# underactuated/HSLabs

Measured on AMD Instinct MI355X. Metric: batched control-loop steps/sec (hexapod.xml, 18-DoF) at 1/2/4/8 MI355X, higher is better.
Workload: dtype f64

## Files before the change

hslabs_amd/api.py:

```python
from __future__ import annotations

import ctypes
from dataclasses import dataclass, field

import numpy as np

from . import capi

GAIT_DTYPE = np.dtype([
    ("torso_pos", "<f8", (3,)), ("torso_angles", "<f8", (3,)), ("step_duration", "<f8"),
    ("period", "<f8"), ("step_length", "<f8"), ("step_height", "<f8"), ("curvature", "<f8"),
    ("foot_shift", "<f8"), ("foot_shift_type", "<i4"), ("rec_transform_flag", "<i4"),
    ("rec_transl", "<f8", (3,)), ("rec_eas", "<f8", (3,)), ("reserved", "<f8", (5,)),
])
assert GAIT_DTYPE.itemsize == 192


def _require(ok: bool, msg: str) -> None:
    if not ok:
        raise ValueError(msg)


def _torch_stream(device, stream):
    import torch
# ... 51 lines not shown
        r["step_length"] = self.step_length
        r["step_height"] = self.step_height
        r["curvature"] = self.curvature
        r["foot_shift_type"] = self.foot_shift[0]
        r["foot_shift"] = self.foot_shift[1]
        if self.rec_transform is not None:
            r["rec_transform_flag"] = 1
            r["rec_transl"] = self.rec_transform[0]
            r["rec_eas"] = self.rec_transform[1]
        return r

    @staticmethod
    def from_record(r) -> "PgsConfigParams":
        return PgsConfigParams(
            torso_pos=tuple(float(v) for v in r["torso_pos"]),
            torso_angles=tuple(float(v) for v in r["torso_angles"]),
            step_duration=float(r["step_duration"]), period=float(r["period"]),
            step_length=float(r["step_length"]), step_height=float(r["step_height"]),
            curvature=float(r["curvature"]), foot_shift=(int(r["foot_shift_type"]), float(r["foot_shift"])),
            rec_transform=((tuple(float(v) for v in r["rec_transl"]), tuple(float(v) for v in r["rec_eas"]))
                           if int(r["rec_transform_flag"]) else None))


def read_pgs_config(path: str, setup_id: int) -> PgsConfigParams:
    L = capi.load()
    c = capi.GaitParamsC()
    buf = ctypes.create_string_buffer(256)
    capi.check(L.hs_pgs_config_read(path.encode(), setup_id, ctypes.byref(c), buf, 256), "hs_pgs_config_read")
    rec = np.frombuffer(bytes(c), dtype=GAIT_DTYPE)[0]
    p = PgsConfigParams.from_record(rec)
    p.fname = buf.value.decode()
    return p


@dataclass
class KinematicModel:

    xml_path: str
    lik_variant: int = -1
    handle: ctypes.c_void_p = field(default=None, repr=False)

    def __post_init__(self):
        L = capi.load()
        h = ctypes.c_void_p()
        capi.check(L.hs_model_load_ex(self.xml_path.encode(), self.lik_variant, ctypes.byref(h)),
                   f"hs_model_load({self.xml_path})")
        self.handle = h
        d = capi.ModelDimsC()
        capi.check(L.hs_model_get_dims(h, ctypes.byref(d)), "hs_model_get_dims")
        self.n_parts, self.nmj, self.nfeet = d.n_parts, d.nmj, d.nfeet
        self.config_dim, self.n_limbs, self.lik_kind = d.config_dim, d.n_limbs, d.lik_kind
        self.total_mass, self.rcap = d.total_mass, d.rcap
        ok = ctypes.c_int32()
        capi.check(L.hs_model_limb_lane(h, ctypes.byref(ok)), "hs_model_limb_lane")
        self.limb_lane_ok = bool(ok.value)

    def get_config_dim(self) -> int:
        return self.config_dim

    def switch_torso_penalty(self, force: bool, torque: bool):
        capi.check(capi.load().hs_model_set_torso_penalty(self.handle, int(bool(force)), int(bool(torque))),
                   "hs_model_set_torso_penalty")

    def torso_penalty(self) -> tuple:
        f, t = ctypes.c_int32(), ctypes.c_int32()
        capi.check(capi.load().hs_model_get_torso_penalty(self.handle, ctypes.byref(f), ctypes.byref(t)),
                   "hs_model_get_torso_penalty")
        return bool(f.value), bool(t.value)

    def number_of_motor_joints(self) -> int:
        return self.nmj

    def get_mnode(self, i: int) -> dict:
        c = capi.NodeInfoC()
        capi.check(capi.load().hs_model_get_node(self.handle, i, ctypes.byref(c)), "hs_model_get_node")
        return {"parent": c.parent, "jtype": c.jtype, "hinge": c.hinge, "foot": c.foot, "limb": c.limb,
                "kids": list(c.kids[:c.n_kids]), "com": np.array(c.com), "foot_pos": np.array(c.foot_pos),
                "mass": c.mass}

    def pergen_rec(self, params, times) -> np.ndarray:
        arr = params_array(params)
        t = np.ascontiguousarray(times, dtype=np.float64).reshape(-1)
        rec = np.zeros((len(arr), len(t), 6 + 3 * self.n_limbs))
        dp = ctypes.POINTER(ctypes.c_double)
        capi.check(capi.load().hs_pergen_rec_host(self.handle, arr.ctypes.data_as(ctypes.POINTER(capi.GaitParamsC)),
                                                  len(arr), t.ctypes.data_as(dp), len(t), rec.ctypes.data_as(dp)),
                   "hs_pergen_rec_host")
        return rec

    def set_jvalues_with_lik(self, rec, ignore_reach: bool = False, config=None):
        r = np.ascontiguousarray(rec, dtype=np.float64).reshape(-1, 6 + 3 * self.n_limbs)
        n = len(r)
        q = np.zeros((n, self.config_dim)) if config is None else np.array(config, np.float64).reshape(n, -1)
        st = np.zeros(n, np.uint32)
        dp = ctypes.POINTER(ctypes.c_double)
        capi.check(capi.load().hs_model_lik_host(self.handle, n, r.ctypes.data_as(dp), int(ignore_reach),
                                                 q.ctypes.data_as(dp), st.ctypes.data_as(ctypes.POINTER(ctypes.c_uint32))),
                   "hs_model_lik_host")
        return q, st

    def recompute_modelnodes(self, config, joints: bool = False):
        q = np.ascontiguousarray(config, dtype=np.float64).reshape(-1, self.config_dim)
        n = len(q)
        ag = np.zeros((n, self.n_parts, 12))
        aj = np.zeros((n, self.n_parts, 12)) if joints else None
        dp = ctypes.POINTER(ctypes.c_double)
        capi.check(capi.load().hs_model_fk_host(self.handle, n, q.ctypes.data_as(dp), self.config_dim,
                                                ag.ctypes.data_as(dp), None if aj is None else aj.ctypes.data_as(dp)),
                   "hs_model_fk_host")

        def rows(a):
            return a.reshape(n, self.n_parts, 4, 3).transpose(0, 1, 3, 2).copy()
        return (rows(ag), rows(aj)) if joints else rows(ag)

    def __del__(self):
        try:
            if self.handle:
                capi.load().hs_model_free(self.handle)
                self.handle = None
        except Exception:
            pass


def limb_tile_launches() -> int:
    return int(capi.load().hs_limb_tile_launches())


def limb_tile_plan_launches() -> int:
    return int(capi.load().hs_limb_tile_plan_launches())


def limb_tile_loop_launches() -> int:
    return int(capi.load().hs_limb_tile_loop_launches())


def limb_launches() -> int:
    return int(capi.load().hs_limb_launches())


def limb_deferred() -> int:
    d = ctypes.c_int64()
    capi.check(capi.load().hs_limb_stats(None, ctypes.byref(d)), "hs_limb_stats")
    return int(d.value)


def limb_tables(model, rollout: int, n_rows: int, device=None, stream=None) -> dict:
    out = dict(ktab=np.zeros((n_rows, 6, 3)), kvel=np.zeros((n_rows, 6, 3)), kbig=np.zeros((n_rows, 6), np.uint8),
               kbad=np.zeros((n_rows, 6), np.uint8))
    dt = ctypes.c_double()
    capi.check(capi.load().hs_debug_limb_tables(model.handle, _cuda_stream(device, stream), rollout, n_rows,
                                                *(out[k].ctypes.data for k in ("ktab", "kvel", "kbig", "kbad")),
                                                ctypes.addressof(dt)), "hs_debug_limb_tables")
    out["dt"] = float(dt.value)
    return out


def params_array(params) -> np.ndarray:
    if isinstance(params, np.ndarray) and params.dtype == GAIT_DTYPE:
        return np.ascontiguousarray(params)
    arr = np.zeros(len(params), GAIT_DTYPE)
    for i, p in enumerate(params):
        arr[i] = p.to_record()
    return arr


def run_host(model: KinematicModel, params, n_t: int = 20, k0: int = 0, horizon: int | None = None,
             ignore_reach: bool = True, want=("q", "tau", "cf", "x", "flags", "work_cot")) -> dict:
    arr = params_array(params)
    B = len(arr)
    H = n_t if horizon is None else horizon
    shapes = _out_shapes(model, B, H)
    out = {k: np.zeros(shapes[k], np.uint32 if k == "flags" else np.float64) if k in want else None
           for k in ("q", "tau", "cf", "x", "flags", "work_cot")}
    dp = ctypes.POINTER(ctypes.c_double)

    def P(a, t=dp):
        return None if a is None else a.ctypes.data_as(t)

    L = capi.load()
    rc = L.hs_run_host(model.handle, arr.ctypes.data_as(ctypes.POINTER(capi.GaitParamsC)), B, n_t, k0, H,
                       int(ignore_reach), P(out["q"]), P(out["tau"]), P(out["cf"]), P(out["x"]),
                       P(out["flags"], ctypes.POINTER(ctypes.c_uint32)), P(out["work_cot"]))
    capi.check(rc, "hs_run_host")
    return out


class ShardedBatch:

    def __init__(self, model: KinematicModel, params, horizon: int = 1, n_t: int = 20, fp32: bool = False,
                 device_mask: int = 1):
        self.model = model
        self.params = params_array(params)
        self.B, self.H, self.n_t = len(self.params), horizon, n_t
        self.dtype = np.float32 if fp32 else np.float64
        L = capi.load()
        h = ctypes.c_void_p()
        capi.check(L.hs_batch_create(model.handle, self.B, horizon, n_t, capi.HS_PREC_F32 if fp32 else capi.HS_PREC_F64,
                                     device_mask, ctypes.byref(h)), "hs_batch_create")
        self.handle = h
        capi.check(L.hs_batch_set_params(h, self.params.ctypes.data_as(ctypes.POINTER(capi.GaitParamsC))),
                   "hs_batch_set_params")

    def _shapes(self) -> dict:
        shapes = _out_shapes(self.model, self.B, self.H)
        return {k: shapes[k] for k, _ in capi.BatchOutputsC._fields_}

    def run(self, k0: int = 0, ignore_reach: bool = True, want=("tau", "cf", "flags", "work", "cot")) -> dict:
        shapes = self._shapes()
        out = {k: np.zeros(shapes[k], np.uint32 if k == "flags" else self.dtype) for k in want}
        o = capi.BatchOutputsC(**{k: v.ctypes.data for k, v in out.items()})
        capi.check(capi.load().hs_batch_run(self.handle, k0, int(ignore_reach), ctypes.byref(o)), "hs_batch_run")
        return out

    def run_device(self, out: dict, k0: int = 0, ignore_reach: bool = True) -> None:
        import torch

        shapes = self._shapes()
        fdt = torch.float32 if self.dtype == np.float32 else torch.float64
        for k, v in out.items():
            if k not in shapes:
                raise ValueError(f"run_device: unknown output {k!r} (expected one of {sorted(shapes)})")
            if not isinstance(v, torch.Tensor) or not v.is_cuda:
                raise ValueError(f"run_device: {k} must be a GPU tensor")
            want = (torch.int32, torch.uint32) if k == "flags" else (fdt,)
            if v.dtype not in want:
                raise ValueError(f"run_device: {k} has dtype {v.dtype}, expected {' or '.join(map(str, want))}")
            if tuple(v.shape) != shapes[k]:
                raise ValueError(f"run_device: {k} has shape {tuple(v.shape)}, expected {shapes[k]}")
            if not v.is_contiguous():
                raise ValueError(f"run_device: {k} must be contiguous")
        o = capi.BatchOutputsC(**{k: v.data_ptr() for k, v in out.items()})
        capi.check(capi.load().hs_batch_run_device(self.handle, k0, int(ignore_reach), ctypes.byref(o)),
                   "hs_batch_run_device")

    def select_best(self, comm: "Comm | None" = None):
        c, i = ctypes.c_float(), ctypes.c_int64()
        L = capi.load()
        if comm is None:
            capi.check(L.hs_select_best(self.handle, ctypes.byref(c), ctypes.byref(i)), "hs_select_best")
        else:
            capi.check(L.hs_select_best_comm(self.handle, comm.handle, ctypes.byref(c), ctypes.byref(i)),
                       "hs_select_best_comm")
        return c.value, i.value

    def __del__(self):
        h = getattr(self, "handle", None)
        if h and capi._lib is not None:
            capi._lib.hs_batch_free(h)
            self.handle = None


class Comm:

    def __init__(self, n_ranks: int, rank: int, uid: bytes):
        _require(len(uid) == capi.COMM_ID_BYTES, f"a comm id is {capi.COMM_ID_BYTES} bytes")
        h = ctypes.c_void_p()
        capi.check(capi.load().hs_comm_init(n_ranks, rank, uid, ctypes.byref(h)), "hs_comm_init")
        self.handle, self.n_ranks, self.rank = h, n_ranks, rank

    @staticmethod
    def unique_id() -> bytes:
        buf = ctypes.create_string_buffer(capi.COMM_ID_BYTES)
        capi.check(capi.load().hs_comm_unique_id(buf), "hs_comm_unique_id")
        return buf.raw

    def reduce_best(self, key, stream=None) -> None:
        capi.check(capi.load().hs_comm_reduce_best(self.handle, key.data_ptr(), _cuda_stream(key.device, stream)),
                   "hs_comm_reduce_best")

    def free(self) -> None:
        if self.handle:
            capi.load().hs_comm_free(self.handle)
            self.handle = None

    def __del__(self):
        try:
            self.free()
        except Exception:
            pass


class DeviceBatch:

    def __init__(self, model: KinematicModel, params, n_t: int = 20, k0: int = 0, horizon: int = 1,
                 ignore_reach: bool = True, outputs=("tau", "cf", "work_cot", "flags"), device=None,
                 rollout_id_base: int = 0, dtype=None):
        import torch

        self.torch = torch
        self.model = model
        self._alloc(model, params, n_t, k0, horizon, ignore_reach, outputs, device, rollout_id_base, dtype)

    def _alloc(self, dims, params, n_t, k0, horizon, ignore_reach, outputs, device, rollout_id_base, dtype=None):
        torch = self.torch
        arr = params_array(params)
        self.B, self.H, self.n_t, self.k0 = len(arr), horizon, n_t, k0
        self.ignore_reach = ignore_reach
        self.rollout_id_base = rollout_id_base
        dev = device or torch.device("cuda", torch.cuda.current_device())
        self.device = dev
        self.dtype = dtype or torch.float64
        self.precision = _precision(self.dtype)
        self.params = torch.from_numpy(arr.view(np.uint8).copy()).to(dev)
        shapes = _out_shapes(dims, self.B, self.H)
        for k in ("q", "dq", "tau", "cf", "x", "flags", "work_cot"):
            setattr(self, k, torch.empty(shapes[k], dtype=torch.int32 if k == "flags" else self.dtype, device=dev)
# ... 663 lines not shown
```

hslabs_amd/capi.py:

```python
from __future__ import annotations

import ctypes
import hashlib
import os

from . import build as _build

ABI_VERSION = 16

HS_OK = 0
HS_FLAG_RANK_RETRY = 1
HS_FLAG_FULL_RANK = 2
HS_FLAG_LOOP_EXHAUST = 4
HS_FLAG_NAN = 8
HS_FLAG_UNREACH = 16
HS_FLAG_NO_CONTACT = 32
HS_FLAG_GENERAL = 64
HS_FLAG_NEAR_RANK = 256
HS_FLAG_DEPENDENT = 512
HS_PREC_F64 = 0
HS_PREC_F32 = 1
HS_SOLVE_AUTO = 0
HS_SOLVE_REFERENCE = 1
KEY_MIN_STEP_LENGTH = 1e-3
COMM_ID_BYTES = 128

EXPORTS = [
    "hs_model_load", "hs_model_load_ex", "hs_model_free", "hs_model_get_dims", "hs_pgs_config_read",
    "hs_run", "hs_run_steps", "hs_run_calls", "hs_run_pd", "hs_run_forces", "hs_run_forces_calls", "hs_mixed_create", "hs_mixed_free",
    "hs_mixed_get_dims", "hs_complete_traj", "hs_traj_save", "hs_run_forces_host",
    "hs_run_mixed", "hs_run_mixed_steps", "hs_run_mixed_calls", "hs_run_host", "hs_best_key_cot", "hs_best_key_encode",
    "hs_best_key_decode", "hs_last_error", "hs_abi_version",
    "hs_sim_default_params", "hs_sim_reset", "hs_sim_step", "hs_sim_create", "hs_sim_advance", "hs_sim_get_state",
    "hs_sim_free", "hs_sim_trial", "hs_sim_trial_summary", "hs_sim_set_trial", "hs_sim_get_trial_state",
    "hs_sim_config", "hs_sim_track_push", "hs_sim_probe", "hs_sim_estimate_workspace",
    "hs_cpc_default_params", "hs_cpc_torques", "hs_cpc_target_points", "hs_sim_cpc_workspace", "hs_sim_cpc_step",
    "hs_batch_create", "hs_batch_set_params", "hs_batch_run", "hs_batch_run_device", "hs_select_best",
    "hs_batch_best_key_device", "hs_batch_free", "hs_comm_unique_id", "hs_comm_init", "hs_comm_free", "hs_comm_size",
    "hs_comm_reduce_best", "hs_select_best_comm", "hs_pergen_rec", "hs_pergen_rec_host", "hs_model_lik",
    "hs_model_lik_host", "hs_model_fk", "hs_model_fk_host", "hs_model_get_node", "hs_model_set_torso_penalty",
    "hs_model_get_torso_penalty", "hs_model_limb_lane", "hs_limb_launches", "hs_limb_tile_launches", "hs_limb_stats",
    "hs_limb_tile_plan_launches", "hs_limb_tile_loop_launches", "hs_debug_limb_tables",
]
EXPORTS_B = ["hs_sim_regress_B", "hs_sim_estimate_B"]
HS_FLAG_LIK_FAILED = 128
SIM_BODY_STRIDE = 13
HS_TRIAL_RUNNING = -1
HS_TRIAL_SURVIVED = -2
HS_CPC_FLAG_NONFINITE = 1
HS_CPC_FLAG_NOSCORE = 2
HS_CPC_FLAG_RANK = 4


class GaitParamsC(ctypes.Structure):

    _fields_ = [
        ("torso_pos", ctypes.c_double * 3),
        ("torso_angles", ctypes.c_double * 3),
        ("step_duration", ctypes.c_double),
        ("period", ctypes.c_double),
        ("step_length", ctypes.c_double),
        ("step_height", ctypes.c_double),
        ("curvature", ctypes.c_double),
        ("foot_shift", ctypes.c_double),
        ("foot_shift_type", ctypes.c_int32),
        ("rec_transform_flag", ctypes.c_int32),
        ("rec_transl", ctypes.c_double * 3),
        ("rec_eas", ctypes.c_double * 3),
        ("reserved", ctypes.c_double * 5),
    ]


assert ctypes.sizeof(GaitParamsC) == 192


class BatchOutputsC(ctypes.Structure):

    _fields_ = [(f, ctypes.c_void_p) for f in ("q", "tau", "cf", "x", "flags", "work", "cot")]


class ModelDimsC(ctypes.Structure):
    _fields_ = [
        ("n_parts", ctypes.c_int32), ("nmj", ctypes.c_int32), ("nfeet", ctypes.c_int32),
        ("config_dim", ctypes.c_int32), ("n_limbs", ctypes.c_int32), ("lik_kind", ctypes.c_int32),
        ("total_mass", ctypes.c_double), ("rcap", ctypes.c_double),
    ]


class NodeInfoC(ctypes.Structure):
    _fields_ = [(f, ctypes.c_int32) for f in ("parent", "jtype", "hinge", "foot", "limb", "n_kids")] + \
               [("kids", ctypes.c_int32 * 6), ("com", ctypes.c_double * 3), ("foot_pos", ctypes.c_double * 3),
                ("mass", ctypes.c_double)]


class PdArgsC(ctypes.Structure):
    _fields_ = [("q_meas", ctypes.c_void_p), ("dq_meas", ctypes.c_void_p), ("k", ctypes.c_double),
                ("tau_cmd", ctypes.c_void_p), ("q_target", ctypes.c_void_p), ("dq_target", ctypes.c_void_p)]


class RunArgsC(ctypes.Structure):
    _fields_ = [
        ("n_rollouts", ctypes.c_int32), ("horizon", ctypes.c_int32), ("k0", ctypes.c_int32),
        ("n_t", ctypes.c_int32), ("ignore_reach", ctypes.c_int32), ("accumulate", ctypes.c_int32),
        ("params", ctypes.c_void_p), ("q", ctypes.c_void_p), ("tau", ctypes.c_void_p),
        ("cf", ctypes.c_void_p), ("x", ctypes.c_void_p), ("flags", ctypes.c_void_p),
        ("work_cot", ctypes.c_void_p), ("best_key", ctypes.c_void_p),
        ("rollout_id_base", ctypes.c_int64), ("stream", ctypes.c_void_p), ("dq", ctypes.c_void_p),
        ("precision", ctypes.c_int32), ("solve_mode", ctypes.c_int32), ("key_steps", ctypes.c_int32),
    ]


class SimParamsC(ctypes.Structure):
    _fields_ = [(f, ctypes.c_double) for f in ("dt", "k", "sor_w", "erp", "cfm", "gravity", "bounce", "bounce_vel",
                                               "soft_cfm", "mu")] + [("iterations", ctypes.c_int32),
                                                                     ("reserved", ctypes.c_int32)]


class SimArgsC(ctypes.Structure):
    _fields_ = [("n_rollouts", ctypes.c_int32), ("n_steps", ctypes.c_int32), ("n_t", ctypes.c_int32),
                ("precision", ctypes.c_int32), ("params", SimParamsC)] + \
               [(f, ctypes.c_void_p) for f in ("body", "seed", "tsi", "q_tab", "dq_tab", "tau_tab", "tau_cmd", "q_meas",
                                               "torso", "n_contacts", "normal_force", "stream")]


class SimTrialArgsC(ctypes.Structure):
    _fields_ = [("sim", SimArgsC)] + \
               [(f, ctypes.c_int32) for f in ("open_loop", "kick_every", "kick_phase", "check_from", "check_until",
                                              "reserved")] + \
               [("torque_limit", ctypes.c_double), ("hc", ctypes.c_double), ("kick_dv", ctypes.c_void_p),
                ("state", ctypes.c_void_p), ("fall_z", ctypes.c_void_p)]


class SimProbeArgsC(ctypes.Structure):
    _fields_ = [("n_rollouts", ctypes.c_int32), ("m", ctypes.c_int32), ("precision", ctypes.c_int32),
                ("reserved", ctypes.c_int32), ("params", SimParamsC)] + \
               [(f, ctypes.c_void_p) for f in ("body", "seed", "tau0", "dtau", "config_out", "tau_out", "body_out",
                                               "n_contacts", "stream")]


class SimEstimateArgsC(ctypes.Structure):
    _fields_ = [("probe", SimProbeArgsC)] + \
               [(f, ctypes.c_void_p) for f in ("ders", "U", "Bt", "rank", "workspace")] + \
               [("workspace_bytes", ctypes.c_size_t)]


class CpcParamsC(ctypes.Structure):
    _fields_ = [(f, ctypes.c_double) for f in ("w", "sg", "k0", "kc", "tauc", "loss_cc", "tp_dist")] + \
               [("n_cand", ctypes.c_int32), ("goal_t0s", ctypes.c_int32), ("tpdist_switch", ctypes.c_int32),
                ("mask", ctypes.c_uint32)]


class CpcArgsC(ctypes.Structure):
    _fields_ = [("n_rollouts", ctypes.c_int32), ("n_tp", ctypes.c_int32), ("precision", ctypes.c_int32),
                ("reserved", ctypes.c_int32), ("params", CpcParamsC), ("Bt", ctypes.c_void_p),
                ("state", ctypes.c_void_p), ("state_stride", ctypes.c_int64), ("tp", ctypes.c_void_p),
                ("tp_stride", ctypes.c_int64)] + \
               [(f, ctypes.c_void_p) for f in ("low_tpdist", "tau", "last_tpi", "flags", "loss", "cand_tpi", "cand_t0s",
                                               "passes", "i_best", "stream")]


class SimCpcArgsC(ctypes.Structure):
    _fields_ = [("trial", SimTrialArgsC), ("cpc", CpcParamsC), ("m", ctypes.c_int32), ("n_tp", ctypes.c_int32),
                ("dtau", ctypes.c_void_p), ("dtau_step_stride", ctypes.c_int64), ("tp", ctypes.c_void_p),
                ("tp_stride", ctypes.c_int64)] + \
               [(f, ctypes.c_void_p) for f in ("ders", "tau0", "low_tpdist", "last_tpi", "flags", "rank", "workspace")] + \
               [("workspace_bytes", ctypes.c_size_t)]


class TrialSummaryC(ctypes.Structure):
    _fields_ = [("running", ctypes.c_int32), ("survived", ctypes.c_int32), ("fallen", ctypes.c_int32),
                ("min_fall_tsi", ctypes.c_int32), ("sum_fall_tsi", ctypes.c_int64)]


C_STRUCTS = {
    "hs_gait_params": GaitParamsC, "hs_model_dims": ModelDimsC, "hs_node_info": NodeInfoC, "hs_run_args": RunArgsC,
    "hs_pd_args": PdArgsC, "hs_batch_outputs": BatchOutputsC, "hs_sim_params": SimParamsC, "hs_sim_args": SimArgsC,
    "hs_sim_trial_args": SimTrialArgsC, "hs_trial_summary": TrialSummaryC, "hs_sim_probe_args": SimProbeArgsC,
    "hs_sim_estimate_args": SimEstimateArgsC, "hs_cpc_params": CpcParamsC, "hs_cpc_args": CpcArgsC,
    "hs_sim_cpc_args": SimCpcArgsC,
}


class HSError(RuntimeError):
    pass


_lib = None
LOADED = None


def lib_path() -> str:
    return _build.LIB


def load(build_if_missing: bool = True) -> ctypes.CDLL:
    global _lib
    if _lib is not None:
        return _lib
    try:
        import torch
    except ImportError:
        pass
    path = _build.LIB
    variant = os.environ.get("HSLABS_VARIANT")
    if variant:
        if not variant.replace("_", "").isalnum():
            raise HSError(f"bad HSLABS_VARIANT {variant!r}")
        path = os.path.join(_build.VARIANT_DIR, f"libhslabs_{variant}.so")
        if not os.path.exists(path):
            raise HSError(f"HSLABS_VARIANT={variant}: {path} not built")
    if not os.path.exists(path):
        if not build_if_missing:
            raise HSError(f"libhslabs.so not built ({path}); run `python -m hslabs_amd.build`")
        _build.build()
    L = ctypes.CDLL(path)
    global LOADED
    with open(path, "rb") as f:
        LOADED = {"path": os.path.relpath(path, os.path.dirname(_build.HERE)),
                  "sha256": hashlib.sha256(f.read()).hexdigest()[:16]}
    dp = ctypes.POINTER(ctypes.c_double)
    vp = ctypes.c_void_p
    L.hs_model_load.argtypes = [ctypes.c_char_p, ctypes.POINTER(vp)]
    L.hs_model_load_ex.argtypes = [ctypes.c_char_p, ctypes.c_int, ctypes.POINTER(vp)]
    L.hs_model_free.argtypes = [vp]
    L.hs_model_free.restype = None
    L.hs_model_get_dims.argtypes = [vp, ctypes.POINTER(ModelDimsC)]
    L.hs_model_set_torso_penalty.argtypes = [vp, ctypes.c_int32, ctypes.c_int32]
    L.hs_model_get_torso_penalty.argtypes = [vp, ctypes.POINTER(ctypes.c_int32), ctypes.POINTER(ctypes.c_int32)]
    L.hs_pgs_config_read.argtypes = [ctypes.c_char_p, ctypes.c_int, ctypes.POINTER(GaitParamsC),
                                     ctypes.c_char_p, ctypes.c_int32]
    L.hs_run.argtypes = [vp, ctypes.POINTER(RunArgsC)]
    L.hs_run_steps.argtypes = [vp, ctypes.POINTER(RunArgsC), ctypes.c_int32, ctypes.POINTER(vp)]
    L.hs_run_calls.argtypes = [vp, ctypes.POINTER(RunArgsC), ctypes.c_int32]
    L.hs_run_mixed_calls.argtypes = [vp, ctypes.POINTER(RunArgsC), ctypes.c_int32]
    L.hs_run_forces.argtypes = [vp, ctypes.POINTER(RunArgsC), vp]
    L.hs_run_forces_calls.argtypes = [vp, ctypes.POINTER(RunArgsC), ctypes.c_int32, vp]
    L.hs_run_forces_host.argtypes = [vp, ctypes.POINTER(GaitParamsC), ctypes.c_int32, ctypes.c_int32, ctypes.c_int32,
                                     ctypes.c_int32, ctypes.c_int32, ctypes.POINTER(ctypes.c_double),
                                     ctypes.POINTER(ctypes.c_double), ctypes.POINTER(ctypes.c_uint32)]
    L.hs_run_pd.argtypes = [vp, ctypes.POINTER(RunArgsC), ctypes.POINTER(PdArgsC)]
    L.hs_complete_traj.argtypes = [vp, ctypes.POINTER(GaitParamsC), ctypes.c_int32, ctypes.c_int32, ctypes.c_int32,
                                   ctypes.POINTER(ctypes.c_double)]
    L.hs_traj_save.argtypes = [ctypes.c_char_p, ctypes.POINTER(ctypes.c_double), ctypes.c_int32, ctypes.c_int32,
                               ctypes.c_int32]
    L.hs_mixed_create.argtypes = [ctypes.POINTER(vp), ctypes.c_int32, ctypes.POINTER(ctypes.c_int32), ctypes.c_int32,
                                  ctypes.POINTER(vp)]
    L.hs_mixed_free.argtypes = [vp]
    L.hs_mixed_free.restype = None
    L.hs_mixed_get_dims.argtypes = [vp, ctypes.POINTER(ModelDimsC)]
    L.hs_run_mixed.argtypes = [vp, ctypes.POINTER(RunArgsC)]
    L.hs_run_mixed_steps.argtypes = [vp, ctypes.POINTER(RunArgsC), ctypes.c_int32, ctypes.POINTER(vp)]
    L.hs_run_host.argtypes = [vp, ctypes.POINTER(GaitParamsC), ctypes.c_int32, ctypes.c_int32, ctypes.c_int32,
                              ctypes.c_int32, ctypes.c_int32, dp, dp, dp, dp, ctypes.POINTER(ctypes.c_uint32), dp]
    L.hs_best_key_cot.argtypes = [ctypes.c_double, ctypes.c_double, ctypes.c_double, ctypes.c_int32, ctypes.c_int32]
    L.hs_best_key_cot.restype = ctypes.c_double
    L.hs_best_key_encode.argtypes = [ctypes.c_double, ctypes.c_int64]
    L.hs_best_key_encode.restype = ctypes.c_uint64
    L.hs_best_key_decode.argtypes = [ctypes.c_uint64, ctypes.POINTER(ctypes.c_float), ctypes.POINTER(ctypes.c_int64)]
    L.hs_best_key_decode.restype = None
    L.hs_sim_default_params.argtypes = [ctypes.POINTER(SimParamsC)]
    L.hs_sim_default_params.restype = None
    L.hs_sim_reset.argtypes = [vp, ctypes.c_int32, vp, ctypes.c_int32, vp, ctypes.c_int32, vp]
    L.hs_sim_step.argtypes = [vp, ctypes.POINTER(SimArgsC)]
    L.hs_sim_create.argtypes = [vp, ctypes.POINTER(GaitParamsC), ctypes.c_int32, ctypes.POINTER(SimParamsC),
                                ctypes.c_double, ctypes.POINTER(vp)]
    L.hs_sim_advance.argtypes = [vp, ctypes.c_int32, dp, dp, dp, ctypes.POINTER(ctypes.c_int32), dp]
    L.hs_sim_get_state.argtypes = [vp, dp, ctypes.POINTER(ctypes.c_int32)]
    L.hs_sim_free.argtypes = [vp]
    L.hs_sim_trial.argtypes = [vp, ctypes.POINTER(SimTrialArgsC)]
    L.hs_sim_trial_summary.argtypes = [vp, ctypes.c_int32, ctypes.POINTER(TrialSummaryC), vp]
    L.hs_sim_set_trial.argtypes = [vp, ctypes.c_int32, ctypes.c_double, ctypes.c_int32, ctypes.c_int32, dp,
                                   ctypes.c_double, ctypes.c_int32, ctypes.c_int32]
    L.hs_sim_get_trial_state.argtypes = [vp, ctypes.POINTER(ctypes.c_int32)]
    L.hs_sim_free.restype = None
    L.hs_sim_config.argtypes = [vp, ctypes.c_int32, vp, vp, ctypes.c_int32, ctypes.c_int32, vp]
    L.hs_sim_track_push.argtypes = [vp, ctypes.c_int32, vp, ctypes.c_int32, ctypes.c_double, vp, ctypes.c_int32, vp]
    L.hs_sim_probe.argtypes = [vp, ctypes.POINTER(SimProbeArgsC)]
    L.hs_sim_regress_B.argtypes = [vp, ctypes.c_int32, ctypes.c_int32, vp, vp, vp, vp, ctypes.c_int32, vp]
    L.hs_sim_estimate_workspace.argtypes = [vp, ctypes.c_int32, ctypes.c_int32]
    L.hs_sim_estimate_workspace.restype = ctypes.c_size_t
    L.hs_sim_estimate_B.argtypes = [vp, ctypes.POINTER(SimEstimateArgsC)]
    L.hs_cpc_default_params.argtypes = [ctypes.POINTER(CpcParamsC)]
    L.hs_cpc_default_params.restype = None
    L.hs_cpc_torques.argtypes = [vp, ctypes.POINTER(CpcArgsC)]
    L.hs_cpc_target_points.argtypes = [vp, ctypes.c_int32, ctypes.c_int32, vp, vp, vp, ctypes.c_uint32, vp, vp]
    L.hs_sim_cpc_workspace.argtypes = [vp, ctypes.c_int32, ctypes.c_int32]
    L.hs_sim_cpc_workspace.restype = ctypes.c_size_t
    L.hs_sim_cpc_step.argtypes = [vp, ctypes.POINTER(SimCpcArgsC)]
    L.hs_batch_create.argtypes = [vp, ctypes.c_int32, ctypes.c_int32, ctypes.c_int32, ctypes.c_int32, ctypes.c_uint32,
                                  ctypes.POINTER(vp)]
    L.hs_batch_set_params.argtypes = [vp, ctypes.POINTER(GaitParamsC)]
    L.hs_batch_run.argtypes = [vp, ctypes.c_int32, ctypes.c_int32, ctypes.POINTER(BatchOutputsC)]
    L.hs_batch_run_device.argtypes = [vp, ctypes.c_int32, ctypes.c_int32, ctypes.POINTER(BatchOutputsC)]
    L.hs_select_best.argtypes = [vp, ctypes.POINTER(ctypes.c_float), ctypes.POINTER(ctypes.c_int64)]
    L.hs_select_best_comm.argtypes = [vp, vp, ctypes.POINTER(ctypes.c_float), ctypes.POINTER(ctypes.c_int64)]
    L.hs_comm_unique_id.argtypes = [ctypes.c_char_p]
    L.hs_comm_init.argtypes = [ctypes.c_int32, ctypes.c_int32, ctypes.c_char_p, ctypes.POINTER(vp)]
    L.hs_comm_free.argtypes = [vp]
    L.hs_comm_free.restype = None
    L.hs_comm_size.argtypes = [vp, ctypes.POINTER(ctypes.c_int32), ctypes.POINTER(ctypes.c_int32)]
    L.hs_comm_reduce_best.argtypes = [vp, vp, vp]
    L.hs_batch_best_key_device.argtypes = [vp, ctypes.c_int32]
    L.hs_batch_best_key_device.restype = vp
    L.hs_batch_free.argtypes = [vp]
    L.hs_batch_free.restype = None
    u32p = ctypes.POINTER(ctypes.c_uint32)
    L.hs_pergen_rec.argtypes = [vp, vp, ctypes.c_int32, vp, ctypes.c_int32, vp, vp]
    L.hs_pergen_rec_host.argtypes = [vp, ctypes.POINTER(GaitParamsC), ctypes.c_int32, dp, ctypes.c_int32, dp]
    L.hs_model_lik.argtypes = [vp, ctypes.c_int32, vp, ctypes.c_int32, vp, vp, vp]
    L.hs_model_lik_host.argtypes = [vp, ctypes.c_int32, dp, ctypes.c_int32, dp, u32p]
    L.hs_model_fk.argtypes = [vp, ctypes.c_int32, vp, ctypes.c_int32, vp, vp, vp]
    L.hs_model_fk_host.argtypes = [vp, ctypes.c_int32, dp, ctypes.c_int32, dp, dp]
    L.hs_model_get_node.argtypes = [vp, ctypes.c_int32, ctypes.POINTER(NodeInfoC)]
    L.hs_last_error.argtypes = []
    L.hs_last_error.restype = ctypes.c_char_p
    L.hs_model_limb_lane.argtypes = [vp, ctypes.POINTER(ctypes.c_int32)]
    L.hs_limb_launches.argtypes = []
    L.hs_limb_launches.restype = ctypes.c_int64
    L.hs_limb_tile_launches.argtypes = []
    L.hs_limb_tile_launches.restype = ctypes.c_int64
    L.hs_limb_tile_plan_launches.argtypes = []
    L.hs_limb_tile_plan_launches.restype = ctypes.c_int64
    L.hs_limb_tile_loop_launches.argtypes = []
    L.hs_limb_tile_loop_launches.restype = ctypes.c_int64
    L.hs_debug_limb_tables.argtypes = [vp, vp, ctypes.c_int32, ctypes.c_int32, vp, vp, vp, vp, vp]
    L.hs_debug_limb_tables.restype = ctypes.c_int
    L.hs_limb_stats.argtypes = [ctypes.POINTER(ctypes.c_int64), ctypes.POINTER(ctypes.c_int64)]
    L.hs_abi_version.argtypes = []
    L.hs_abi_version.restype = ctypes.c_int
    if L.hs_abi_version() != ABI_VERSION:
        raise HSError("libhslabs ABI version mismatch")
    _lib = L
    return L


def check(rc: int, what: str = "") -> None:
    if rc != HS_OK:
        msg = load().hs_last_error().decode(errors="replace")
        raise HSError(f"{what}: {msg} (rc={rc})")
```

hslabs_amd/csrc/hs_capi.cpp:

```cpp
#include <hip/hip_runtime.h>

#include <algorithm>
#include <atomic>
#include <cmath>
#include <cstdio>
#include <cstdlib>
#include <cfloat>
#include <cstring>
#include <fstream>
#include <mutex>
#include <string>
#include <vector>

#include "hs_internal.h"

namespace {

thread_local std::string g_err;

int fail(int code, const std::string& msg) {
  g_err = msg;
  return code;
}

// ... 114 lines not shown
    hs_simtopo_t<float> h;
    hs_simtopo_round(h, m->sim);
    hs_simtopo_t<float>* d = nullptr;
    e = hipMalloc(&d, sizeof(h));
    if (e != hipSuccess) return failed(e, "hipMalloc(simtopo f32)");
    e = hipMemcpy(d, &h, sizeof(h), hipMemcpyHostToDevice);
    if (e != hipSuccess) { (void)hipFree(d); return failed(e, "hipMemcpy(simtopo f32)"); }
    m->sim_dev_f32[dev] = d;
  }
  dv.sim = m->sim_dev[dev];
  if (precision == HS_PREC_F32) dv.sim_f32 = m->sim_dev_f32[dev];
  return dv;
}

hs_run_args routed(const hs_run_args& a, int32_t torso_mask) {
  hs_run_args c = a;
  if (torso_mask != 3) c.solve_mode = HS_SOLVE_REFERENCE;
  return c;
}

int check_args(const hs_model_s* m, const hs_run_args* a) {
  if (!m || !a) return fail(HS_E_ARG, "null model or args");
  if (a->n_rollouts < 0) return fail(HS_E_ARG, "n_rollouts < 0");
  if (a->horizon < 1) return fail(HS_E_ARG, "horizon must be >= 1");
  if (a->k0 < 0) return fail(HS_E_ARG, "k0 must be >= 0");
  if (a->precision != HS_PREC_F64 && a->precision != HS_PREC_F32) return fail(HS_E_ARG, "unknown precision");
  if (a->n_t < 1) return fail(HS_E_ARG, "n_t must be >= 1");
  if (a->n_rollouts > 0 && !a->params) return fail(HS_E_ARG, "params is null");
  if (a->n_rollouts > (1 << 30)) return fail(HS_E_ARG, "too many rollouts");
  if (a->solve_mode != HS_SOLVE_AUTO && a->solve_mode != HS_SOLVE_REFERENCE) return fail(HS_E_ARG, "unknown solve_mode");
  if (a->key_steps < 0) return fail(HS_E_ARG, "key_steps < 0");
  if (a->best_key && !a->work_cot) return fail(HS_E_ARG, "best_key needs work_cot (the key is the work's COT)");
  return HS_OK;
}

struct launch_ctx {
  bool empty = false;
  const hs::kernels* k = nullptr;
  const hs_topo* d_topo = nullptr;
  void* ws = nullptr;
  hs::launch_map map{};
  run_pools* pools = nullptr;
  double total_mass = 0.0;
  const double* rollout_mass = nullptr;
  const hs_topo* host = nullptr;
  int32_t torso_mask = 3;
};

template <class Check = int (*)()>
int model_ctx(hs_model_t m, const hs_run_args* a, int32_t n_calls, launch_ctx& cx,
              Check entry_check = [] { return (int)HS_OK; }) {
  int rc = check_args(m, a);
  if (rc != HS_OK) return rc;
  if (n_calls < 0) return fail(HS_E_ARG, "n_calls < 0");
  rc = entry_check();
  if (rc != HS_OK) return rc;
  cx.empty = a->n_rollouts == 0 || n_calls == 0;
  if (cx.empty) return HS_OK;
  rc = device_state(m, a->n_rollouts + 1, a->stream, &cx.d_topo, &cx.ws);
  if (rc != HS_OK) return rc;
  cx.k = &hs::kernels_of(a->precision);
  cx.map = hs::single_model_map(m->host, a->n_rollouts);
  hs::ktab_range(a->k0, a->n_t, a->horizon, n_calls, &cx.map.ktab_lo, &cx.map.ktab_n, &cx.map.ttab_n);
  cx.pools = m;
  cx.total_mass = m->host.total_mass;
  cx.host = &m->host;
  cx.torso_mask = m->host.torso_mask;
  return HS_OK;
}

int mixed_ctx(hs_mixed_t p, const hs_run_args* a, int32_t n_calls, launch_ctx& cx) {
  if (!p) return fail(HS_E_ARG, "null plan");
  int rc = check_args(p->models[0], a);
  if (rc != HS_OK) return rc;
  if (a->n_rollouts != p->n_rollouts) return fail(HS_E_ARG, "n_rollouts differs from the plan's");
  if (n_calls < 0) return fail(HS_E_ARG, "n_calls < 0");
  int dev = 0;
  hipError_t e = hipGetDevice(&dev);
  if (e != hipSuccess) return hip_fail(e, "hipGetDevice");
  if (dev != p->dev) return fail(HS_E_DEVICE, "plan was created on another device");
  cx.empty = a->n_rollouts == 0 || n_calls == 0;
  if (cx.empty) return HS_OK;
  hs::launch_map& mp = cx.map;
  mp.wave_model = p->d_wave_model;
  mp.wave_rollouts = p->d_wave_rollouts;
  mp.n_waves = p->n_waves;
  mp.max_parts = p->max_dims.n_parts;
  mp.st_tau = p->st_tau;
  mp.st_cf = p->st_cf;
  mp.st_q = p->st_q;
  mp.st_x = p->st_x;
  if (p->d_limb_model) {
    mp.limb_model = p->d_limb_model;
    mp.limb_rollouts = p->d_limb_rollouts;
    mp.limb_slots = p->d_limb_rollouts + 8 * (size_t)p->limb_waves;
    mp.limb_waves = p->limb_waves;
  }
  hs::ktab_range(a->k0, a->n_t, a->horizon, n_calls, &mp.ktab_lo, &mp.ktab_n, &mp.ttab_n);
  {
    std::lock_guard<std::mutex> lk(p->mu);
    e = (hipError_t)p->ws.get(a->stream, (size_t)p->n_rollouts + 1, &cx.ws);
  }
  if (e != hipSuccess) return hip_fail(e, "hipMalloc(workspace)");
  cx.k = &hs::kernels_of(a->precision);
  cx.d_topo = p->d_topos;
  cx.pools = p;
  cx.rollout_mass = p->d_rollout_mass;
  cx.host = &p->models[0]->host;
  cx.torso_mask = p->torso_mask;
  return HS_OK;
}

int launch_setup(const launch_ctx& cx, const hs_run_args& c, hs::launch_map& mp) {
  mp.setup_only = 1;
  mp.setup_io = hs::SETUP_STORE;
  const int le = cx.k->launch_fused(cx.d_topo, c, cx.ws, mp);
  mp.setup_only = 0;
  mp.setup_io = hs::SETUP_LOAD;
  mp.fix_n_counts = 0;
  return le;
}

int launch_steps(const launch_ctx& cx, const hs_run_args& a, int32_t n_calls, void* const* kernel_events) {
  const hs::kernels& k = *cx.k;
  hs_run_args c = a;
  hipStream_t st = (hipStream_t)a.stream;
  if (c.key_steps == 0) c.key_steps = (int32_t)std::min<int64_t>((int64_t)n_calls * a.horizon, INT32_MAX);
  const bool key_reduce = a.best_key && a.work_cot && !cx.map.tau_in;
  hs::launch_map mp = cx.map;
  const int le0 = launch_setup(cx, c, mp);
  if (le0 != 0) return hip_fail((hipError_t)le0, "kernel launch (setup pass)");
  for (int32_t i = 0; i < n_calls; i++) {
    c.k0 = (int32_t)(((int64_t)a.k0 + (int64_t)i * a.horizon) % a.n_t);
    c.best_key = (i + 1 == n_calls && !key_reduce) ? a.best_key : nullptr;
    hipError_t e = hipSuccess;
    if (kernel_events) e = hipEventRecord((hipEvent_t)kernel_events[2 * i], st);
    if (e != hipSuccess) return hip_fail(e, "hipEventRecord");
    int le = k.launch_rollouts(cx.d_topo, c, cx.ws, mp);
    if (le != 0) return hip_fail((hipError_t)le, "kernel launch");
    if (kernel_events) e = hipEventRecord((hipEvent_t)kernel_events[2 * i + 1], st);
    if (e != hipSuccess) return hip_fail(e, "hipEventRecord");
  }
  if (key_reduce) {
    hs_run_args r = c;
    r.best_key = a.best_key;
    r.accumulate = 1;
    const int le = k.launch_fused_reduce(r, cx.total_mass, cx.rollout_mass, nullptr, 0);
    if (le != 0) return hip_fail((hipError_t)le, "kernel launch (best key)");
  }
  return HS_OK;
}

std::atomic<int64_t> g_limb_launches{0};
std::atomic<int64_t> g_limb_tile_launches{0};
std::atomic<int64_t> g_limb_tile_plan_launches{0};
std::atomic<int64_t> g_limb_tile_loop_launches{0};
#define HS_ONLINE_MAX_H 64

bool env_switch(const char* name, bool on_by_default) {
  const char* e = getenv(name);
  if (!e) return on_by_default;
  return on_by_default ? e[0] != '0' : e[0] == '1';
}

enum class step_route {
  ROLLOUT,
  ONLINE_DEFER,
  LIMB_ONLINE,
  FUSED,
  LIMB_FUSED,
};
enum class run_entry { STEPS, CALLS, FORCES_CALLS };

step_route route(const launch_ctx& cx, const hs_run_args& a, run_entry entry) {
  const bool forces = entry == run_entry::FORCES_CALLS, f32 = a.precision == HS_PREC_F32;
  const auto limb_eligible = [&] {
    return env_switch("HS_LIMB", true) && cx.host->limb_lane_ok && a.solve_mode == HS_SOLVE_AUTO && !a.q &&
           (forces || (!a.x && !a.dq)) && (!f32 || (!forces && env_switch("HS_LIMB_F32", true)));
  };
  const bool table = cx.map.ktab_n > 0 && (!cx.map.wave_rollouts || cx.map.limb_rollouts);
  if (entry != run_entry::STEPS) return limb_eligible() && table ? step_route::LIMB_FUSED : step_route::FUSED;
  if (a.horizon > HS_ONLINE_MAX_H) return step_route::ROLLOUT;
  if (env_switch("HS_LIMB_ONLINE", false) && limb_eligible())
    return table ? step_route::LIMB_ONLINE : step_route::ONLINE_DEFER;
  if (env_switch("HS_ONLINE_DEFER", false) && a.solve_mode == HS_SOLVE_AUTO) return step_route::ONLINE_DEFER;
  return step_route::ROLLOUT;
}

#ifndef HS_LIMB_TILE_MIN_STEPS
#define HS_LIMB_TILE_MIN_STEPS 40
#endif
bool limb_tile(step_route rt, const hs_run_args& a, int32_t n) {
  if (rt != step_route::LIMB_FUSED || !env_switch("HS_LIMB_TILE", true)) return false;
  if (!limb_tile_desc_ok(n, a.horizon, a.k0, a.n_t)) return false;
  if (const char* e = getenv("HS_LIMB_TILE_MIN")) {
    char* end = nullptr;
    const long min_n = strtol(e, &end, 10);
    if (end != e && *end == '\0' && min_n >= 1) return n >= min_n;
  }
  const int32_t idle = HS_TILE_SLOTS * limb_tile_count(n) - n;
  return a.precision != HS_PREC_F32 && n >= HS_LIMB_TILE_MIN_STEPS && 32 * idle <= n;
}
int32_t limb_tile_plan_mode() {
  if (!env_switch("HS_LIMB_TILE_PLAN", true)) return 0;
  const char* e = getenv("HS_LIMB_TILE_PLAN");
  return e && e[0] == '2' ? 2 : 1;
}
#ifndef HS_LIMB_TILE_LOOP_TILES
#define HS_LIMB_TILE_LOOP_TILES 5
#endif
#ifndef HS_LIMB_TILE_LOOP_ROUNDS
#define HS_LIMB_TILE_LOOP_ROUNDS 4
#endif
constexpr int64_t HS_RESIDENT_LIMB_WAVES = 2048;
int32_t limb_tile_loop(const hs_run_args& a, int32_t n) {
  const int32_t nt = limb_tile_count(n);
  if (a.precision == HS_PREC_F32) return 1;
  if (const char* e = getenv("HS_LIMB_TILE_LOOP")) {
    char* end = nullptr;
    const long tl = strtol(e, &end, 10);
    if (end != e && *end == '\0' && tl >= 1) return (int32_t)std::min<long>(tl, HS_TILE_PLAN_STEPS);
  }
  return limb_tile_loop_rule(nt, a.n_rollouts, HS_LIMB_TILE_LOOP_TILES, HS_LIMB_TILE_LOOP_ROUNDS * HS_RESIDENT_LIMB_WAVES);
}

#ifndef HS_FUSED_WAVES
#define HS_FUSED_WAVES 524288
#endif
#ifndef HS_FUSED_MAX_STEPS
#define HS_FUSED_MAX_STEPS 256
#endif
#ifndef HS_FUSED_RESERVE_STEPS
#define HS_FUSED_RESERVE_STEPS 1024
#endif
int32_t fused_chunk(const hs::launch_map& mp) {
  return std::max(1, std::min(HS_FUSED_MAX_STEPS, HS_FUSED_WAVES / std::max(1, mp.n_waves)));
}

size_t fix_counts_bytes(int32_t n_counts) { return ((size_t)n_counts * sizeof(int32_t) + 255) / 256 * 256; }
size_t fix_bytes(int32_t n_counts, int32_t chunk, const hs::launch_map& mp) {
  return fix_counts_bytes(n_counts) + (size_t)chunk * mp.n_waves * 2 * 2 * sizeof(int32_t);
}
void fix_carve(void* fix, int32_t n_counts, hs::launch_map& mp) {
  mp.fix_count = (int32_t*)fix;
  mp.fix_n_counts = n_counts;
  mp.fix_items = (int32_t*)((char*)fix + fix_counts_bytes(n_counts));
}

int run_fused(const launch_ctx& cx, const hs_run_args& a, int32_t n_calls, step_route rt,
              void* const* kernel_events = nullptr) {
  const bool online = rt == step_route::ONLINE_DEFER || rt == step_route::LIMB_ONLINE;
  const bool limb = rt == step_route::LIMB_ONLINE || rt == step_route::LIMB_FUSED;
  const hs::kernels& k = *cx.k;
  hs::launch_map mp = cx.map;
  const int64_t S = online ? a.horizon : (int64_t)n_calls * a.horizon;
  if (S > (1 << 24) || (int64_t)n_calls * a.horizon > INT32_MAX) return fail(HS_E_ARG, "too many steps");
  const int32_t B = a.n_rollouts;
  const int32_t CHUNK = online ? a.horizon : fused_chunk(mp);
  const int32_t n_chunks = online ? n_calls : (int32_t)((S + CHUNK - 1) / CHUNK);
  const size_t gwb = ws_slot_bytes();
  const int32_t n_counts = 2 * n_chunks;
  void *gen = nullptr, *work = nullptr, *fix = nullptr;
  {
    std::lock_guard<std::mutex> lk(cx.pools->mu);
    hipError_t e = (hipError_t)cx.pools->fused_gen.get(
        a.stream, ((size_t)CHUNK * (B + 1) * hs::solve_workspace_bytes() + gwb - 1) / gwb, &gen);
    const size_t need = (size_t)S * B * sizeof(double);
    const size_t want =
        std::max(need, std::min((size_t)HS_FUSED_RESERVE_STEPS * B * sizeof(double), (size_t)512 << 20));
    if (e == hipSuccess) e = (hipError_t)cx.pools->fused_work.get(a.stream, (want + gwb - 1) / gwb, &work);
    if (e == hipSuccess)
      e = (hipError_t)cx.pools->fused_fix.get(a.stream, (fix_bytes(n_counts, CHUNK, mp) + gwb - 1) / gwb, &fix);
    if (e != hipSuccess) return hip_fail(e, "hipMalloc(fused workspace)");
  }
  int32_t* fix_counts = (int32_t*)fix;
  hs_run_args c = a;
  c.horizon = (int32_t)S;
  c.best_key = nullptr;
  hs_run_args r = a;
  if (r.key_steps == 0) r.key_steps = (int32_t)((int64_t)n_calls * a.horizon);
  mp.fused_h = a.horizon;
  mp.fused_work = work;
  mp.fused_gen = gen;
  fix_carve(fix, n_counts, mp);
  const bool barrier_ok = (B + 63) / 64 <= 1024 && env_switch("HS_FIX_BARRIER", true);
  mp.prep_unit = limb ? 8 : 2;
  mp.ktab_rates = 0;
  for (int32_t i = 0; !online && i < n_chunks; i++)
    mp.ktab_rates |= limb_tile(rt, a, (int32_t)std::min<int64_t>(CHUNK, S - (int64_t)i * CHUNK)) ? 1 : 0;
  int le = launch_setup(cx, c, mp);
  mp.red_total_mass = cx.total_mass;
  mp.red_rollout_mass = cx.rollout_mass;
  mp.red_key_steps = r.key_steps;
  hipStream_t st = (hipStream_t)a.stream;
  for (int32_t i = 0; le == 0 && i < n_chunks; i++) {
    const int64_t s0 = online ? 0 : (int64_t)i * CHUNK;
    const bool last = i + 1 == n_chunks;
    if (online) c.k0 = (int32_t)(((int64_t)a.k0 + (int64_t)i * a.horizon) % a.n_t);
    mp.fused_s0 = (int32_t)s0;
    mp.fused_n = (int32_t)std::min<int64_t>(CHUNK, S - s0);
    mp.fix_mode = hs::FIX_DEFER;
    mp.fix_count = fix_counts + i;
    mp.fix_reduce = 0;
    mp.limb_tile = limb_tile(rt, a, mp.fused_n);
    mp.limb_tile_loop = mp.limb_tile ? limb_tile_loop(a, mp.fused_n) : 1;
    hipError_t e = kernel_events ? hipEventRecord((hipEvent_t)kernel_events[2 * i], st) : hipSuccess;
    if (e != hipSuccess) return hip_fail(e, "hipEventRecord");
    int32_t planned = 0;
    le = limb ? k.launch_limb(cx.d_topo, c, cx.ws, mp, limb_tile_plan_mode(), &planned)
              : k.launch_fused(cx.d_topo, c, cx.ws, mp);
    g_limb_launches += limb;
    g_limb_tile_launches += mp.limb_tile;
    g_limb_tile_plan_launches += planned;
    g_limb_tile_loop_launches += mp.limb_tile && std::min(mp.limb_tile_loop, limb_tile_count(mp.fused_n)) > 1;
    if (le != 0) break;
    mp.fix_mode = hs::FIX_SOLVE;
    mp.fix_reduce = a.work_cot && a.solve_mode == HS_SOLVE_AUTO && (online || last);
    mp.fix_barrier = barrier_ok ? fix_counts + n_chunks + i : nullptr;
    mp.red_n_steps = (int32_t)S;
    mp.red_best_key = last ? r.best_key : nullptr;
    le = k.launch_fused(cx.d_topo, c, cx.ws, mp);
    if (le == 0 && kernel_events) e = hipEventRecord((hipEvent_t)kernel_events[2 * i + 1], st);
    if (e != hipSuccess) return hip_fail(e, "hipEventRecord");
  }
  if (le == 0 && !mp.fix_reduce) le = k.launch_fused_reduce(r, cx.total_mass, cx.rollout_mass, work, (int32_t)S);
  if (le != 0) return hip_fail((hipError_t)le, "kernel launch");
  return HS_OK;
}

}

namespace hs {

launch_map single_model_map(const hs_topo& t, int32_t n_rollouts) {
  launch_map mp{};
  mp.n_waves = (n_rollouts + 1) / 2;
  mp.max_parts = t.n;
  mp.ktab_nl = t.n_limbs;
  mp.st_tau = t.nmj;
  mp.st_cf = 3 * t.nf;
  mp.st_q = t.cfg;
  mp.st_x = 6 * t.n;
  return mp;
}

}

extern "C" {

int hs_abi_version(void) { return HSLABS_ABI_VERSION; }

int hs_model_limb_lane(hs_model_t m, int32_t* ok) {
  if (!m || !ok) return fail(HS_E_ARG, "null argument");
  *ok = m->host.limb_lane_ok;
  return HS_OK;
}

int64_t hs_limb_launches(void) { return g_limb_launches.load(); }
int64_t hs_limb_tile_launches(void) { return g_limb_tile_launches.load(); }
int64_t hs_limb_tile_plan_launches(void) { return g_limb_tile_plan_launches.load(); }
int64_t hs_limb_tile_loop_launches(void) { return g_limb_tile_loop_launches.load(); }

int hs_limb_stats(int64_t* launches, int64_t* deferred) {
  if (launches) *launches = g_limb_launches.load();
  if (deferred) {
    unsigned long long n[2] = {0, 0};
    hipError_t e = (hipError_t)hs::kernels_f64.limb_deferred(&n[0]);
    if (e == hipSuccess) e = (hipError_t)hs::kernels_f32.limb_deferred(&n[1]);
    if (e != hipSuccess) return hip_fail(e, "hs_limb_stats");
    *deferred = (int64_t)(n[0] + n[1]);
  }
  return HS_OK;
}

int hs_debug_limb_tables(hs_model_t m, void* stream, int32_t rollout, int32_t n_rows, double* ktab, double* kvel,
                         uint8_t* kbig, uint8_t* kbad, double* dt) {
  if (!m) return fail(HS_E_ARG, "null argument");
  int dev = 0;
  hipError_t e = hipGetDevice(&dev);
  if (e != hipSuccess) return hip_fail(e, "hipGetDevice");
  const void* ws = nullptr;
  {
    std::lock_guard<std::mutex> lk(m->mu);
    for (const auto& s : m->ws.live)
      if (s.dev == dev && s.stream == stream && rollout >= 0 && (size_t)rollout < s.n) ws = s.ptr;
  }
  if (!ws) return fail(HS_E_ARG, "no workspace of this model, device and stream holds that rollout");
  e = (hipError_t)hs::limb_tables_read(ws, rollout, n_rows, ktab, kvel, kbig, kbad, dt, stream);
  if (e != hipSuccess) return hip_fail(e, "hs_debug_limb_tables");
  return HS_OK;
}

const char* hs_last_error(void) { return g_err.c_str(); }

int hs_model_load_ex(const char* xml_path, int lik_variant, hs_model_t* out) {
  if (!xml_path || !out) return fail(HS_E_ARG, "null argument");
  hs_model_s* m = new hs_model_s;
  memset(m->dev, 0, sizeof(m->dev));
  memset(m->sim_dev, 0, sizeof(m->sim_dev));
  memset(m->sim_dev_f32, 0, sizeof(m->sim_dev_f32));
  std::string err;
  int rc = hs::load_model_file(xml_path, lik_variant, &m->host, err, &m->sim);
  if (rc != HS_OK) {
    delete m;
    return fail(rc, err);
  }
  *out = m;
  return HS_OK;
}

int hs_model_load(const char* xml_path, hs_model_t* out) { return hs_model_load_ex(xml_path, -1, out); }

void hs_model_free(hs_model_t m) {
  if (!m) return;
  for (int d = 0; d < HS_MAX_DEVICES; d++) {
    if (m->dev[d]) free_on_device(d, m->dev[d]);
    if (m->sim_dev[d]) free_on_device(d, m->sim_dev[d]);
    if (m->sim_dev_f32[d]) free_on_device(d, m->sim_dev_f32[d]);
  }
  m->release();
  delete m;
}

int hs_model_get_dims(hs_model_t m, hs_model_dims* o) {
  if (!m || !o) return fail(HS_E_ARG, "null argument");
  const hs_topo& t = m->host;
  o->n_parts = t.n;
  o->nmj = t.nmj;
  o->nfeet = t.nf;
  o->config_dim = t.cfg;
  o->n_limbs = t.n_limbs;
  o->lik_kind = t.lik_kind;
  o->total_mass = t.total_mass;
  o->rcap = t.rcap;
  return HS_OK;
}

int hs_model_set_torso_penalty(hs_model_t m, int32_t force, int32_t torque) {
  if (!m) return fail(HS_E_ARG, "null model");
  if (!force && !torque) return fail(HS_E_ARG, "switch_torso_penalty(0,0): mask0 not set (ftsolver.cpp:245)");
  const int32_t mask = (force ? 1 : 0) | (torque ? 2 : 0);
  std::lock_guard<std::mutex> lk(m->mu);
  m->host.torso_mask = mask;
  bool uploaded = false;
  for (int dev = 0; dev < HS_MAX_DEVICES; dev++) uploaded |= m->dev[dev] != nullptr;
  if (!uploaded) return HS_OK;
  int cur = 0;
  hipError_t e = hipGetDevice(&cur);
  if (e != hipSuccess) return hip_fail(e, "hipGetDevice");
  for (int dev = 0; dev < HS_MAX_DEVICES && e == hipSuccess; dev++) {
    if (!m->dev[dev]) continue;
    e = hipSetDevice(dev);
    if (e == hipSuccess) e = hipDeviceSynchronize();
    if (e == hipSuccess)
      e = hipMemcpy(&m->dev[dev]->torso_mask, &mask, sizeof(mask), hipMemcpyHostToDevice);
  }
  (void)hipSetDevice(cur);
  if (e != hipSuccess) return hip_fail(e, "hs_model_set_torso_penalty");
  return HS_OK;
}

int hs_model_get_torso_penalty(hs_model_t m, int32_t* force, int32_t* torque) {
  if (!m || !force || !torque) return fail(HS_E_ARG, "null argument");
  *force = (m->host.torso_mask & 1) ? 1 : 0;
  *torque = (m->host.torso_mask & 2) ? 1 : 0;
  return HS_OK;
}

int hs_model_get_node(hs_model_t m, int32_t i, hs_node_info* o) {
  if (!m || !o) return fail(HS_E_ARG, "null argument");
  const hs_topo& t = m->host;
  if (i < 0 || i >= t.n) return fail(HS_E_ARG, "node index out of range");
  const hs_node& nd = t.node[i];
  memset(o, 0, sizeof(*o));
  o->parent = nd.parent;
  o->jtype = nd.jtype;
  o->hinge = nd.hinge;
  o->foot = nd.foot;
  o->limb = -1;
  for (int L = 0; L < t.n_limbs; L++)
    if (t.limb_child[L] == i) o->limb = L;
  o->n_kids = nd.nkids;
  for (int k = 0; k < nd.nkids && k < HS_NODE_MAX_KIDS; k++) o->kids[k] = nd.kids[k];
  for (int r = 0; r < 3; r++) {
    o->com[r] = nd.com[r];
    o->foot_pos[r] = nd.foot >= 0 ? nd.cap[r] : 0.0;
  }
  o->mass = t.mass[i];
  return HS_OK;
}

int hs_pgs_config_read(const char* path, int setup_id, hs_gait_params* out, char* xml_file, int32_t xml_file_len) {
  if (!path || !out) return fail(HS_E_ARG, "null argument");
  std::string xml, err;
  int rc = hs::read_pgs_config(path, setup_id, out, xml, err);
  if (rc != HS_OK) return fail(rc, err);
  if (xml_file && xml_file_len > 0) {
    snprintf(xml_file, (size_t)xml_file_len, "%s", xml.c_str());
  }
  return HS_OK;
}

int hs_run(hs_model_t m, const hs_run_args* a) { return hs_run_steps(m, a, 1, nullptr); }

int hs_run_steps(hs_model_t m, const hs_run_args* a, int32_t n_calls, void* const* kernel_events) {
  launch_ctx cx;
  const int rc = model_ctx(m, a, n_calls, cx);
  if (rc != HS_OK || cx.empty) return rc;
  const hs_run_args r = routed(*a, cx.torso_mask);
  const step_route rt = route(cx, r, run_entry::STEPS);
  if (rt == step_route::ROLLOUT) return launch_steps(cx, r, n_calls, kernel_events);
  return run_fused(cx, r, n_calls, rt, kernel_events);
}

int hs_run_calls(hs_model_t m, const hs_run_args* a, int32_t n_calls) {
  launch_ctx cx;
  const int rc = model_ctx(m, a, n_calls, cx);
  if (rc != HS_OK || cx.empty) return rc;
  const hs_run_args r = routed(*a, cx.torso_mask);
  return run_fused(cx, r, n_calls, route(cx, r, run_entry::CALLS));
}

int hs_run_pd(hs_model_t m, const hs_run_args* a, const hs_pd_args* pd) {
  launch_ctx cx;
  const int rc = model_ctx(m, a, 1, cx, [&]() -> int {
    if (!pd || (a->n_rollouts > 0 && (!pd->q_meas || !pd->dq_meas || !pd->tau_cmd)))
      return fail(HS_E_ARG, "pd: q_meas, dq_meas and tau_cmd are required");
    if (!(pd->k >= 0)) return fail(HS_E_ARG, "pd: k must be >= 0");
    return HS_OK;
  });
  if (rc != HS_OK || cx.empty) return rc;
  hs::launch_map& mp = cx.map;
  hs::ktab_range(a->k0, a->n_t, 1, a->horizon, &mp.ktab_lo, &mp.ktab_n, &mp.ttab_n);
  mp.pd_q = pd->q_meas;
  mp.pd_dq = pd->dq_meas;
  mp.pd_k1 = -pd->k;
  mp.pd_k2 = -2 * std::sqrt(pd->k);
  mp.pd_tau = pd->tau_cmd;
  mp.pd_q0 = pd->q_target;
  mp.pd_dq0 = pd->dq_target;
  return launch_steps(cx, routed(*a, cx.torso_mask), 1, nullptr);
}
// ... 1467 lines not shown
```

hslabs_amd/csrc/hs_internal.h:

```cpp
#pragma once
#include <cstddef>
#include <mutex>
#include <string>
#include <vector>

#include "../../include/hslabs.h"
#include "hs_simtopo.h"
#include "hs_limb_tile.h"
#include "hs_topo.h"

struct hs_sim_probe_kargs {
  hs_sim_args sim;
  int32_t m, pad;
  const double* tau0;
  const double* dtau;
  double* config_out;
  double* tau_out;
  double* body_out;
  uint32_t* seed_out;
};

namespace hs {

int set_error(int code, const std::string& msg);
int comm_reduce_min(hs_comm_t comm, uint64_t* key, void* stream);
int comm_device(hs_comm_t comm);
uint64_t* comm_scratch(hs_comm_t comm);

int load_model_file(const char* path, int lik_variant, hs_topo* t, std::string& err, hs_simtopo* sim = nullptr);
int read_pgs_config(const char* path, int setup_id, hs_gait_params* out, std::string& xml, std::string& err);

enum { SETUP_COMPUTE = 0, SETUP_STORE = 1, SETUP_LOAD = 2 };
enum { FIX_NONE = 0, FIX_DEFER = 1, FIX_SOLVE = 2 };

struct launch_map {
  const int32_t* wave_model;
  const int32_t* wave_rollouts;
  int32_t n_waves;
  int32_t max_parts;
  int32_t h_row;
  int32_t setup_io;
  const double* tau_in;
  const double *pd_q, *pd_dq;
  double pd_k1, pd_k2;
  double *pd_tau, *pd_q0, *pd_dq0;
  int32_t st_tau, st_cf, st_q, st_x;
  int32_t fused_w, fused_s0, fused_n, fused_h;
  void* fused_work;
  void* fused_gen;
  int32_t setup_only;
  int32_t fix_mode;
  int32_t* fix_count;
  int32_t* fix_items;
  int32_t fix_n_counts;
  int32_t fix_reduce, red_key_steps, red_n_steps;
  int32_t* fix_barrier;
  double red_total_mass;
  const double* red_rollout_mass;
  uint64_t* red_best_key;
  int32_t ktab_n, ktab_lo, ktab_nl, ttab_n;
  int32_t ktab_rates = 0;
  int32_t prep_unit;
  const int32_t *limb_model, *limb_rollouts, *limb_slots;
  int32_t limb_waves;
  int32_t limb_tile;
  int32_t limb_tile_loop;
};

size_t solve_workspace_bytes();
int limb_tables_read(const void* workspace, int32_t rollout, int32_t n_rows, double* ktab, double* kvel, uint8_t* kbig,
                     uint8_t* kbad, double* dt, void* stream);
void ktab_range(int32_t k0, int32_t n_t, int32_t horizon, int64_t n_calls, int32_t* lo, int32_t* n_table,
                int32_t* n_ttab);
launch_map single_model_map(const hs_topo& t, int32_t n_rollouts);

struct kernels {
  size_t (*general_workspace_bytes)();
  int (*launch_rollouts)(const hs_topo* d_topo, const hs_run_args& a, void* workspace, const launch_map& mp);
  int (*launch_fused)(const hs_topo* d_topo, const hs_run_args& a, void* workspace, const launch_map& mp);
  int (*launch_limb)(const hs_topo* d_topo, const hs_run_args& a, void* workspace, const launch_map& mp,
                     int32_t tile_plan, int32_t* tile_planned);
  int (*launch_fused_reduce)(const hs_run_args& a, double total_mass, const double* rollout_mass,
                             const void* work_steps, int32_t n_steps);
  int (*limb_deferred)(unsigned long long* out);
};
extern const kernels kernels_f64, kernels_f32;
inline const kernels& kernels_of(int32_t precision) { return precision == HS_PREC_F32 ? kernels_f32 : kernels_f64; }

int launch_pergen_rec(const hs_topo* d_topo, const hs_gait_params* params, int32_t n_rollouts, const double* times,
                      int32_t n_times, double* rec, void* stream);
int launch_fk(const hs_topo* d_topo, int32_t n_parts, int32_t n_cfg, const double* config, int32_t stride,
              double* a_ground, double* a_joint, void* stream);
int launch_lik(const hs_topo* d_topo, int32_t n_cfg, const double* rec, int32_t ignore_reach, double* config,
               uint32_t* status, void* stream);

struct sim_dev {
  const hs_topo* topo;
  const hs_simtopo* sim;
  const hs_simtopo_t<float>* sim_f32;
  const hs_simtopo& host;
};
int launch_sim_reset(const sim_dev& dv, int32_t n_rollouts, const double* config, int32_t config_stride, double* body,
                     int32_t precision, void* stream);
int launch_sim_steps(const sim_dev& dv, const hs_sim_args& a);
int launch_sim_trial(const sim_dev& dv, const hs_sim_trial_args& a);
int launch_trial_summary(const int32_t* state, int32_t n, hs_trial_summary* acc, void* stream);
int sim_step_occupancy(int32_t n, int32_t m_max, int32_t* out3);
int launch_sim_config(const sim_dev& dv, int32_t n, const double* body, double* config, int32_t config_stride,
                      int32_t precision, void* stream);
int launch_track_push(int32_t n, int32_t cfg, const double* config, int32_t config_stride, double dt, double* ders,
                      void* stream);
int launch_sim_probe(const sim_dev& dv, const hs_sim_probe_kargs& a);
int launch_probe_accel(int32_t n, int32_t m, int32_t cfg, const double* config_out, const double* ders, double dt,
                       double* U, void* stream);
int launch_regress_B(int32_t n, int32_t m, int32_t nmj, int32_t cfg, const double* T, const double* U, double* Bt,
                     int32_t* rank, void* stream);
size_t regress_lds_bytes(int32_t m, int32_t nmj, int32_t cfg);
size_t cpc_lds_bytes(int32_t n_tp, int32_t n_cand, int32_t nmj, int32_t cfg);
int launch_cpc_torques(const hs_cpc_args& a, int32_t nmj, int32_t cfg);
int launch_cpc_target_points(int32_t n, int32_t n_t, int32_t cfg, int32_t nmj, const double* q_tab, const double* dq_tab,
                             const double* tau_tab, uint32_t mask, double* tp, void* stream);
int launch_cpc_rows(int32_t n, int32_t width, const int32_t* state, const double* src, double* dst, void* stream);
int launch_cpc_keep_seed(int32_t n, const int32_t* state, const uint32_t* saved, uint32_t* seed, void* stream);

}

constexpr int HS_MAX_DEVICES = 64;

struct ws_pool {
  struct slot {
    int dev;
    void* stream;
    void* ptr;
    size_t n;
  };
  std::vector<slot> live;
  std::vector<std::pair<int, void*>> retired;
  int get(void* stream, size_t n, void** out);
  void release();
};

struct run_pools {
  ws_pool ws;
  ws_pool fused_gen, fused_work;
  ws_pool fused_fix;
  std::mutex mu;
  void release() {
    for (ws_pool* p : {&ws, &fused_gen, &fused_work, &fused_fix}) p->release();
  }
};

struct hs_model_s : run_pools {
  hs_topo host;
  hs_topo* dev[HS_MAX_DEVICES];
  hs_simtopo sim;
  hs_simtopo* sim_dev[HS_MAX_DEVICES];
  hs_simtopo_t<float>* sim_dev_f32[HS_MAX_DEVICES];
};
```

hslabs_amd/csrc/hs_kernels.hip:

```cpp
#include "hs_rollout_kernel.h"
#include "hs_limb.h"

namespace {

__global__ __launch_bounds__(WAVE) void hs_pergen_rec_kernel(const hs_topo* __restrict__ T,
                                                             const hs_gait_params* __restrict__ params,
                                                             int32_t n_rollouts, const double* __restrict__ times,
                                                             int32_t n_times, double* __restrict__ rec) {
  __shared__ SetupL st[2];
  const int sub = threadIdx.x / HALF, lane = threadIdx.x % HALF;
  const int64_t n_items = (int64_t)n_rollouts * n_times;
  const int64_t item = (int64_t)blockIdx.x * 2 + sub;
  const bool live = item < n_items;
  const int64_t it = live ? item : n_items - 1;
  const int b = (int)(it / n_times), ti = (int)(it % n_times);
  const GaitR g = load_gait(params[b]);
  gait_setup(T, g, 1, st[sub], lane);
  const int nl = T->n_limbs;
  if (live && lane < nl) {
    real o0[3], o1[3], target[3];
    bool turned;
    gait_record<false>(g, params[b], limb_rec(st[sub], T->limb_pergen[lane]), (real)times[ti], o0, o1, turned, target);
    double* r = rec + it * (6 + 3 * nl);
    if (lane == 0)
      for (int i = 0; i < 3; i++) { r[i] = o0[i]; r[3 + i] = o1[i]; }
    for (int i = 0; i < 3; i++) r[6 + 3 * lane + i] = target[i];
  }
}

}

#ifdef HS_DBG
extern "C" int hs_debug_read_dbg(double* out, int n) {
  if (n > (1 << 22)) n = 1 << 22;
  return (int)hipMemcpyFromSymbol(out, HIP_SYMBOL(g_dbg), sizeof(double) * n, 0, hipMemcpyDeviceToHost);
}
#endif

#ifdef HS_STAMPS
extern "C" int hs_debug_read_stamps(unsigned long long* out, int n_rows) {
  if (n_rows > 4096) n_rows = 4096;
  return (int)hipMemcpyFromSymbol(out, HIP_SYMBOL(g_stamps), sizeof(unsigned long long) * 32 * n_rows, 0,
                                  hipMemcpyDeviceToHost);
}
extern "C" int hs_debug_set_stamp_base(unsigned int base) {
  return (int)hipMemcpyToSymbol(HIP_SYMBOL(g_stamp_base), &base, sizeof(base), 0, hipMemcpyHostToDevice);
}
extern "C" int hs_debug_set_stamp_iter(int iter) {
  return (int)hipMemcpyToSymbol(HIP_SYMBOL(g_stamp_iter), &iter, sizeof(iter), 0, hipMemcpyHostToDevice);
}
extern "C" int hs_debug_clear_stamps() {
  static unsigned long long zero[4096][32];
  return (int)hipMemcpyToSymbol(HIP_SYMBOL(g_stamps), zero, sizeof(zero), 0, hipMemcpyHostToDevice);
}
#endif

namespace hs {

size_t solve_workspace_bytes() { return sizeof(SolveWS); }

int limb_tables_read(const void* workspace, int32_t rollout, int32_t n_rows, double* ktab, double* kvel, uint8_t* kbig,
                     uint8_t* kbad, double* dt, void* stream) {
  static_assert(std::is_same<real, double>::value, "the fp64 unit's RolloutWS");
  if (n_rows < 0 || n_rows > HS_KTAB) return (int)hipErrorInvalidValue;
  const RolloutWS* W = (const RolloutWS*)workspace + rollout;
  hipError_t e = hipStreamSynchronize((hipStream_t)stream);
  const auto get = [&](void* dst, const void* src, size_t n) {
    if (e == hipSuccess && dst && n) e = hipMemcpy(dst, src, n, hipMemcpyDeviceToHost);
  };
  get(ktab, W->ktab, sizeof(W->ktab[0]) * n_rows);
  get(kvel, W->kvel, sizeof(W->kvel[0]) * n_rows);
  get(kbig, W->kbig, sizeof(W->kbig[0]) * n_rows);
  get(kbad, W->kbad, sizeof(W->kbad[0]) * n_rows);
  get(dt, &W->st.dt, sizeof(double));
  return (int)e;
}

void ktab_range(int32_t k0, int32_t n_t, int32_t horizon, int64_t n_calls, int32_t* lo_out, int32_t* n_out,
                int32_t* ttab_out) {
  int64_t lo = INT64_MAX, hi = 0;
  const int64_t nc = n_calls < n_t ? n_calls : n_t;
  for (int64_t c = 0; c < nc; c++) {
    const int64_t f = ((int64_t)k0 + c * horizon) % n_t;
    lo = f < lo ? f : lo;
    hi = f + horizon + NS - 1 > hi ? f + horizon + NS - 1 : hi;
  }
  const int64_t n = nc > 0 ? hi - lo : 0;
  *lo_out = nc > 0 ? (int32_t)lo : 0;
  *n_out = n <= HS_KTAB ? (int32_t)n : 0;
  *ttab_out = (int32_t)(n < HS_KTAB ? n : HS_KTAB);
}

int launch_pergen_rec(const hs_topo* d_topo, const hs_gait_params* params, int32_t n_rollouts, const double* times,
                      int32_t n_times, double* rec, void* stream) {
  const int64_t items = (int64_t)n_rollouts * n_times;
  if (items <= 0) return 0;
  hipLaunchKernelGGL(hs_pergen_rec_kernel, dim3((unsigned)((items + 1) / 2)), dim3(WAVE), 0, (hipStream_t)stream,
                     d_topo, params, n_rollouts, times, n_times, rec);
  return (int)hipGetLastError();
}

#ifndef __HIP_DEVICE_COMPILE__
extern const kernels kernels_f64 = {general_workspace_bytes, launch_rollouts,     launch_fused,
                                    launch_limb,             launch_fused_reduce, limb_deferred};
#endif

}
```

hslabs_amd/csrc/hs_kernels_f32.hip:

```cpp
#define HS_REAL float
#define HS_REAL_IS_FLOAT 1
#include "hs_rollout_kernel.h"
#include "hs_limb.h"

namespace hs {

#ifndef __HIP_DEVICE_COMPILE__
extern const kernels kernels_f32 = {general_workspace_bytes, launch_rollouts,     launch_fused,
                                    launch_limb,             launch_fused_reduce, limb_deferred};
#endif

}
```

hslabs_amd/csrc/hs_limb.h:

```cpp
#pragma once
#include "hs_limb_tile.h"
#include "hs_step_base.h"
#include "hs_step_kin.h"
#include "hs_step_solve.h"

namespace {

#ifndef HS_LIMB_WAVES
#define HS_LIMB_WAVES 2
#endif
#ifndef HS_LIMB_WAVES_F32
#define HS_LIMB_WAVES_F32 HS_LIMB_WAVES
#endif

constexpr int LG = 8;
constexpr int LGR = WAVE / LG;

__device__ inline int dbg_row(bool live, int b, int horizon, int s_glob) { return live ? b * horizon + s_glob : -1; }
#ifdef HS_DBG
#define LDBG(dbg_r, slot, val, n)                                                                                \
  do {                                                                                                           \
    if (HS_DBG == (n) && (dbg_r) >= 0 && (size_t)(dbg_r) * 32 + (slot) < (1u << 22)) g_dbg[(size_t)(dbg_r) * 32 + (slot)] = (double)(val); \
  } while (0)
#else
#define LDBG(dbg_r, slot, val, n) do {} while (0)
#endif

__device__ unsigned long long g_limb_deferred;

template <int NM, bool FORCES = false>
struct LimbLds {
  real g[NM][6];
  real a[6];
  real wd[HS_NMAX];
  real p[FORCES ? NM : 1][3];
};

__device__ inline real grp_get(real v, int src) { return __shfl(v, src); }
__device__ inline float grp_getf(float v, int src) { return __shfl(v, src); }
__device__ inline bool grp_any(bool p, int gbase) { return ((__ballot(p) >> gbase) & 0xFFull) != 0; }
__device__ inline uint32_t grp_or(uint32_t v) {
  v |= (uint32_t)__shfl_xor((int)v, 1);
  v |= (uint32_t)__shfl_xor((int)v, 2);
  v |= (uint32_t)__shfl_xor((int)v, 4);
  return v;
}
__device__ inline real rank8_sum(real v) {
  v += dpp_r<0xB1>(v);
  v += dpp_r<0x4E>(v);
  v += dpp_r<0x141>(v);
  return v;
}


__device__ inline const hs_topo* opaque_s(const hs_topo* p) {
  using gptr = const __attribute__((address_space(1))) hs_topo*;
  gptr q = (gptr)p;
  asm volatile("" : "+s"(q));
  return (const hs_topo*)q;
}

template <bool CENTRE>
__device__ __attribute__((always_inline)) inline void fk_link(const hs_topo* T, const hs_link& lk, int kk, A34& Jv,
                                                              A34& H, real s, real c, real* P, real* U, real* Jp,
                                                              real* Jz, real* fp, bool& contact) {
  if (kk > 0) Jv = mul(H, load34(lk.P));
  H = mul_hinge(Jv, c, s);
  {
    const real cm[3] = {(real)lk.com[0], (real)lk.com[1], (real)lk.com[2]};
    mulp(H, cm, P);
  }
  {
    real R[9];
#pragma unroll
    for (int i = 0; i < 9; i++) R[i] = (real)lk.Rpj[i];
    auto a_rc = [&](int r, int c) { return H(r, 0) * R[c * 3 + 0] + H(r, 1) * R[c * 3 + 1] + H(r, 2) * R[c * 3 + 2]; };
    U[0] = (a_rc(2, 1) - a_rc(1, 2)) / 2;
    U[1] = (a_rc(0, 2) - a_rc(2, 0)) / 2;
    U[2] = (a_rc(1, 0) - a_rc(0, 1)) / 2;
  }
  if (CENTRE) {
#pragma unroll
    for (int i = 0; i < 3; i++) Jp[i] = Jv(i, 3);
#pragma unroll
    for (int i = 0; i < 3; i++) Jz[i] = Jv(i, 2);
    if (kk == 2) {
      const real cp[3] = {(real)lk.cap[0], (real)lk.cap[1], (real)lk.cap[2]};
      mulp(H, cp, fp);
      contact = fp[2] < (real)(T->rcap + 1e-4);
    }
  }
}

__device__ inline void part_dyn(real m, real inv, const real* Pm, const real* P0, const real* Pp, const real* Um,
                                const real* U0, const real* Up, real* f) {
  real vp[3], vm[3], mr[3], wp[3], wm[3], amr[3];
  for (int j = 0; j < 3; j++) {
    vp[j] = Pp[j] - P0[j];
    vp[j] *= inv;
    vm[j] = P0[j] - Pm[j];
    vm[j] *= inv;
    real mp = vp[j] * m, mm = vm[j] * m;
    mr[j] = mp - mm;
    mr[j] *= inv;
    wp[j] = Up[j] - U0[j];
    wp[j] *= inv;
    wm[j] = U0[j] - Um[j];
    wm[j] *= inv;
  }
  for (int j = 0; j < 3; j++) {
    amr[j] = wp[j] - wm[j];
    amr[j] *= inv;
  }
  for (int j = 0; j < 3; j++) {
    f[j] = mr[j];
    f[3 + j] = amr[j];
  }
  opaque_vals<6>(f);
  f[2] += m * real(1);
}

__device__ inline void part_g(const real* P, const real* o, real* f) {
  opaque_vals<6>(f);
  real d[3];
  for (int j = 0; j < 3; j++) d[j] = P[j] - o[j];
  f[3] += d[1] * f[2] - d[2] * f[1];
  f[4] += d[2] * f[0] - d[0] * f[2];
  f[5] += d[0] * f[1] - d[1] * f[0];
  opaque_vals<6>(f);
}

struct BodyS {
  real P[3], U[3];
};
__device__ inline BodyS body_straight(const real* bf, const real* u, real tv) {
  BodyS s;
  for (int i = 0; i < 3; i++) s.P[i] = fma(tv, u[i], bf[i]);
  for (int i = 0; i < 3; i++) s.U[i] = bf[3 + i];
  return s;
}
__device__ inline BodyS body_frame(const A34& A, const real* com) {
  BodyS s;
  mulp(A, com, s.P);
  s.U[0] = (A(2, 1) - A(1, 2)) / 2;
  s.U[1] = (A(0, 2) - A(2, 0)) / 2;
  s.U[2] = (A(1, 0) - A(0, 1)) / 2;
  return s;
}

__device__ __attribute__((always_inline)) inline A34 limb_frame(const hs_topo* T, int L, bool straight, const bool own,
                                                                const RolloutWS& W, const KinFrames& kf, int row,
                                                                const real* u, real tv, BodyS& ob) {
  if (straight) {
    if (own) ob = body_straight(kf.own[L][0], u, tv);
    return frame_at(load34r(kf.J0[L]), u, tv);
  }
  A34 A = load34r(W.ktor[row] + 6);
  const int clen = T->limb_chain_len[L];
  for (int kk = 1; kk < clen; kk++) {
    const int v = T->limb_chain[L][kk];
    A = mul(A, node_pj(T, v));
    if (T->node[v].owner_limb == L) {
      const real com[3] = {(real)T->node[v].com[0], (real)T->node[v].com[1], (real)T->node[v].com[2]};
      ob = body_frame(A, com);
    }
  }
  return mul(A, node_joint_parent(T, T->limb_child[L]));
}

__device__ __attribute__((always_inline)) inline void limb_outer(const hs_topo* T, const hs_link (&LK)[3], const A34& J,
                                                                 const real* ja, real (&P)[3][3], real (&U)[3][3],
                                                                 bool& big) {
  real sq[3], cq[3];
#pragma unroll
  for (int kk = 0; kk < 3; kk++) {
    big |= sincos_big(ja[kk]);
    sincos_k_small(ja[kk], &sq[kk], &cq[kk]);
  }
  A34 Jv = J, H;
  real nul[3];
  bool nc = false;
#pragma unroll
  for (int kk = 0; kk < 3; kk++) fk_link<false>(T, LK[kk], kk, Jv, H, sq[kk], cq[kk], P[kk], U[kk], nul, nul, nul, nc);
}

__device__ __attribute__((always_inline)) inline void outer_put(real (&outer)[36][LGR * HS_LMAX], int o0, int col,
                                                                const real (&P)[3][3], const real (&U)[3][3]) {
#pragma unroll
  for (int kk = 0; kk < 3; kk++)
#pragma unroll
    for (int j = 0; j < 3; j++) {
      outer[o0 + 3 * kk + j][col] = P[kk][j];
      outer[o0 + 9 + 3 * kk + j][col] = U[kk][j];
    }
}
__device__ __attribute__((always_inline)) inline void outer_get(const real (&outer)[36][LGR * HS_LMAX], int kk, int col,
                                                                real* Pm, real* Um, real* Pp, real* Up) {
#pragma unroll
  for (int j = 0; j < 3; j++) {
    Pm[j] = outer[3 * kk + j][col];
    Um[j] = outer[9 + 3 * kk + j][col];
    Pp[j] = outer[18 + 3 * kk + j][col];
    Up[j] = outer[27 + 3 * kk + j][col];
  }
}

__device__ inline bool limb_rows_big(const real* qm, const real* q0, const real* qp) {
  bool big = false;
#pragma unroll
  for (int kk = 0; kk < 3; kk++) big |= sincos_big(qm[kk]);
#pragma unroll
  for (int kk = 0; kk < 3; kk++) big |= sincos_big(q0[kk]);
#pragma unroll
  for (int kk = 0; kk < 3; kk++) big |= sincos_big(qp[kk]);
  return big;
}

__device__ inline void limb_defer(const hs::launch_map& mp, bool live, int l, int s_glob, int item) {
  if (l == 0 && live) {
    atomicAdd(&g_limb_deferred, 1ull);
    const int it = atomicAdd(mp.fix_count, 1);
    mp.fix_items[2 * it] = s_glob - mp.fused_s0;
    mp.fix_items[2 * it + 1] = item;
  }
}

__device__ inline int rank_limb(const hs_topo* T, uint32_t cm, int nl, int rank) {
  int src = 0;
  for (int L2 = 0; L2 < nl; L2++) {
    const int f2 = T->link[L2][2].foot;
    if (((cm >> f2) & 1) && __popc(cm & ((1u << f2) - 1)) == rank) src = L2;
  }
  return src;
}

__device__ __attribute__((always_inline)) inline void contact_block(const real (&Jp)[3][3], const real (&Jz)[3][3],
                                                                    const real (&xt)[3][3], const real* fp, real* Dp6,
                                                                    real* gc) {
  real tD[3][6], tg[3][3];
#pragma unroll
  for (int m = 0; m < 3; m++) {
    const int p = 2 - m;
    real Dp[6] = {0, 0, 0, 0, 0, 0}, g[3] = {0, 0, 0};
    real da[3], va[3][3];
    for (int r = 0; r < 3; r++) da[r] = Jp[p][r] - fp[r];
    cross_rows(da, va);
#pragma unroll
    for (int r = 0; r < 3; r++) {
      const real w2 = Jz[p][r] * Jz[p][r];
#pragma unroll
      for (int i = 0; i < 3; i++) {
        if (i == r) continue;
#pragma unroll
        for (int j = 0; j <= i; j++)
          if (j != r) Dp[i * (i + 1) / 2 + j] += w2 * va[r][i] * va[r][j];
        g[i] += w2 * va[r][i] * xt[p][r];
      }
    }
    for (int e = 0; e < 6; e++) tD[m][e] = Dp[e];
    for (int i = 0; i < 3; i++) tg[m][i] = g[i];
  }
#pragma unroll
  for (int e = 0; e < 6; e++) Dp6[e] = (tD[0][e] + tD[1][e]) + (tD[2][e] + real(0));
#pragma unroll
  for (int i = 0; i < 3; i++) gc[i] = (tg[0][i] + tg[1][i]) + (tg[2][i] + real(0));
}

template <int NM>
__device__ __attribute__((always_inline)) inline void limb_forces(const hs_topo* T, const hs_run_args& a,
                                                                  const hs::launch_map& mp, LimbLds<NM, true>& S, bool limb,
                                                                  int l, int L, int gbase, int nl, bool live, int b,
                                                                  int s_glob, const real* o,
                                                                  const real (&Jp)[3][3], const real (&Jz)[3][3],
                                                                  const real (&Pc)[3][3], const real* fp,
                                                                  const real (&xt)[3][3], bool bad, bool big) {
  const int n = T->n;
  [[maybe_unused]] const int dbg_r = dbg_row(live, b, a.horizon, s_glob);
  real ts[9];
#pragma unroll
  for (int q = 0; q < 9; q++) ts[q] = 0;
  for (int i = 1; i < n; i++) {
    real r[3];
    for (int t = 0; t < 3; t++) r[t] = S.p[i][t] - o[t];
    real q[6] = {r[0] * r[0], r[1] * r[1], r[2] * r[2], r[0] * r[1], r[0] * r[2], r[1] * r[2]};
    opaque_vals<6>(q);
    ts[0] += r[0];
    ts[1] += r[1];
    ts[2] += r[2];
    for (int j = 0; j < 6; j++) ts[3 + j] += q[j];
  }
  opaque_vals<9>(ts);
  const int dbg_f = T->link[L][2].foot;
  (void)dbg_f;
  if (l == 0) LDBG(dbg_r, 0, ts[3], 30);
  const size_t orow = (size_t)b * a.horizon + s_glob;
  real Ct[18], Bd[6], Bl[9], rdB[3], rb[3], vl[27];
  bool okB = true;
  if (limb) {
    const real* z = inp(mp.tau_in) + (live ? orow : 0) * mp.st_tau;
    real zz[3];
    for (int kk = 0; kk < 3; kk++) zz[kk] = z[T->node[T->limb_node[L][kk]].hinge];
    ForcesRows F;
    forces_rows(F, Jp, Jz, Pc, fp, o, xt, zz);
    okB = forces_foot(F, fp, o, Ct, Bd, Bl, rdB, rb);
    LDBG(dbg_r, 24 + dbg_f, Ct[0], 36);
    LDBG(dbg_r, 24 + dbg_f, rb[0], 37);
    if (okB) {
      ForcesV G;
      forces_v(G, Ct, Bl, rdB, rb);
#pragma unroll
      for (int e = 0; e < 27; e++) {
        const TriWalk<> t(e < 21 ? e : 0);
        real pa = e < 21 ? F.prod(t.r, t.c) : F.prod(e - 21, 9);
        real pb = e < 21 ? G.vprod(t.r, t.c) : G.vprod(e - 21, 6);
        opaque_vals<1>(&pa);
        opaque_vals<1>(&pb);
        vl[e] = (e < 21) ? pb - pa : pb + pa;
      }
    }
  }
  const bool fast = !grp_any(limb && !okB, gbase);
  if (!fast || grp_any(big, gbase)) {
    limb_defer(mp, live, l, s_glob, b);
    return;
  }
  real kv[27];
#pragma unroll
  for (int e = 0; e < 27; e++) {
    const real v = limb ? vl[e] : real(0);
    real s = real(0) + v;
    for (int k = 1; k < nl; k++) {
      const real prev = dpp_r<0x111>(s);
      if (l >= 1) s = prev + v;
    }
    const real tot = grp_get(s, gbase + nl - 1);
    const real dtv = (e < 21) ? real(0) : (e < 24 ? S.a[e - 21] : S.a[e - 21]);
// ... 66 lines not shown
  }
  __device__ real mass(int L, int kk) const {
    if constexpr (LOOP) return k[L].m[kk];
    else return (real)T->mass[T->limb_node[L][kk]];
  }
  __device__ real mass_own(int L) const {
    if constexpr (LOOP) return k[L].mown;
    else return (real)T->mass[T->limb_own[L][0]];
  }
  __device__ int hinge(int L, int kk) const {
    if constexpr (LOOP) return (k[L].hf >> (8 * kk)) & 255;
    else return T->link[L][kk].hinge;
  }
  __device__ int foot(int L) const {
    if constexpr (LOOP) return k[L].hf >> 24;
    else return T->link[L][2].foot;
  }
  __device__ int kid(int l) const {
    if constexpr (LOOP) return k[l].kid & 255;
    else return T->node[0].kids[l];
  }
  __device__ int kid_size(int l, int c) const {
    if constexpr (LOOP) return (k[l].kid >> 8) & 255;
    else return T->node[c].size;
  }
};


__device__ inline const limb_tile_entry& limb_tile_entry_of(const limb_tile_desc& d, int tile) { return d.tile[tile]; }
static_assert(HS_LMAX < LG, "lane LG - 1 of a group must not be a limb lane (lane_push's idle target)");
__device__ inline real lane_push(real v, int dst) {
  if constexpr (sizeof(real) == 8) {
    const double d = (double)v;
    const int lo = __builtin_amdgcn_ds_permute(dst << 2, __double2loint(d));
    const int hi = __builtin_amdgcn_ds_permute(dst << 2, __double2hiint(d));
    return (real)__hiloint2double(hi, lo);
  } else {
    return (real)__int_as_float(__builtin_amdgcn_ds_permute(dst << 2, __float_as_int((float)v)));
  }
}

struct LimbKD {
  real g3[3][6];
  real Jp[3][3], Jz[3][3], fp[3];
  bool contact = false;
  bool own = false;
  real gown[6];
  real jvel[3];
  real Pc[3][3], Pown[3];
  bool bad = false, big = false;
};

template <bool FORCES, bool BARRIER, bool LOOP>
__device__ __attribute__((always_inline)) inline void limb_centre_link(
    const LimbModelK<LOOP>& mk, const real (&outer)[36][LGR * HS_LMAX], int ol, int l, int L, int kk, real* P0, real* U0,
    real* Jp, real* Jz, real* fp, real* Pc, const real* o, real inv, real* g, int dbg_r) {
  opaque_vals<3>(P0);
  if constexpr (FORCES)
    for (int j = 0; j < 3; j++) Pc[j] = P0[j];
  opaque_vals<3>(U0);
  opaque_vals<3>(Jp);
  opaque_vals<3>(Jz);
  if (kk == 2) opaque_vals<3>(fp);
  real Pm[3], Um[3], Pp[3], Up[3];
  if constexpr (BARRIER) __builtin_amdgcn_sched_barrier(0);
  outer_get(outer, kk, ol, Pm, Um, Pp, Up);
  part_dyn(mk.mass(L, kk), inv, Pm, P0, Pp, Um, U0, Up, g);
  [[maybe_unused]] const int node = mk.node(L, kk);
  LDBG(dbg_r, node, P0[0], 1);
  LDBG(dbg_r, node, U0[0], 5);
  LDBG(dbg_r, node, g[0], 2);
  LDBG(dbg_r, node, g[3], 10);
  LDBG(dbg_r, node, g[1], 13);
  LDBG(dbg_r, node, g[2], 14);
  LDBG(dbg_r, node, g[4], 16);
  if (l == 0) LDBG(dbg_r, 31, o[0], 15);
  if (l == 0) LDBG(dbg_r, 30, o[1], 15);
  LDBG(dbg_r, node, Um[0], 9);
  LDBG(dbg_r, node, Up[0], 11);
  LDBG(dbg_r, node, Pm[0], 12);
  part_g(P0, o, g);
  LDBG(dbg_r, node, g[3], 3);
}

struct LimbTileRates {
  real v[3];
  uint32_t big0, big2, big4, bad;
  __device__ __attribute__((always_inline)) inline void issue(const RolloutWS& W, int row0, int L) {
#pragma unroll
    for (int kk = 0; kk < 3; kk++) v[kk] = W.kvel[row0 + 2][L][kk];
    big0 = W.kbig[row0][L];
    big2 = W.kbig[row0 + 2][L];
    big4 = W.kbig[row0 + 4][L];
    bad = W.kbad[row0 + 2][L];
  }
  __device__ __attribute__((always_inline)) inline void finish(LimbKD& kd) {
    asm volatile("" : "+v"(big0), "+v"(big2), "+v"(big4), "+v"(bad));
    kd.bad = bad != 0;
    kd.big |= (big0 | big2 | big4) != 0;
#pragma unroll
    for (int kk = 0; kk < 3; kk++) kd.jvel[kk] = v[kk];
  }
};

#ifdef HS_STAMPS
#undef HS_STAMP_GATE
#define HS_STAMP_GATE stamp_on
#endif
template <bool FORCES, bool LOOP>
__device__ __attribute__((always_inline)) inline void limb_tile_kd(
    const hs_topo* T_, const LimbModelK<LOOP>& mk, const KinFrames& kf, const real* ttab,
    real (&outer)[36][LGR * HS_LMAX], hs_link (&links)[HS_LMAX][3], const RolloutWS& W, bool straight,
    const real* u, real v, int lane, int nl, bool limb, int L, bool live, int row0, uint32_t M, uint64_t req,
    const real* tv, const real* o, real inv, real dt, LimbKD& kd, int dbg_r, bool stamp_on) {
  (void)dbg_r;
  (void)stamp_on;
  const int grp = lane >> 3, l = lane & 7;
  const bool shm = live && !((M >> (2 * grp)) & 1);
  const bool shp = live && !((M >> (2 * grp + 1)) & 1);
  const int nreq = __popc(M);
  auto nth_req = [req](int r) { return (int)(req >> (4 * r)) & 15; };
  const int nidle = LG - nl;
  const int E0 = (LGR * nidle) / nl;
  const int rqm = __popc(M & ((1u << (2 * grp)) - 1)), rqp = __popc(M & ((1u << (2 * grp + 1)) - 1));
  const int pm = shm || rqm < E0 ? 0 : 1 + (rqm - E0) / LGR, pp = shp || rqp < E0 ? 0 : 1 + (rqp - E0) / LGR;
  auto col = [](int ln) { return (ln >> 3) * HS_LMAX + (ln & 7); };
  real P[3][3], U[3][3];
  BodyS om, op, oc;
  kd.own = limb && mk.own(L);
  [[maybe_unused]] LimbTileRates tr;
  {
    int rq = 0, fL = L;
    bool extra = false;
    if (!limb) {
      const int j = grp * nidle + (l - nl);
      rq = j / nl;
      fL = j - rq * nl;
      extra = rq < E0 && rq < nreq;
      if (!extra) rq = 0, fL = 0;
    }
    const int bit = nth_req(rq), gr = bit >> 1, side = bit & 1;
    const int rr = __shfl(row0, gr * LG);
    const int frow = limb ? row0 + 2 : rr + 4 * side;
    const int dst = gr * LG + fL;
    const int dm = limb ? (shp ? lane + LG : -1) : (extra && side == 0 ? dst : -1);
    const int dp = limb ? (shm ? lane - LG : -1) : (extra && side == 1 ? dst : -1);
    BodyS ob;
#pragma unroll
    for (int j = 0; j < 3; j++) ob.P[j] = ob.U[j] = real(0);
    if (limb || extra) {
      const hs_topo* T = opaque_s(T_);
      const bool fown = LimbModelK<LOOP>{T, mk.k}.own(fL);
      const real tvf = LOOP && limb ? tv[2] : ttab[frow] * v;
      const A34 J = limb_frame(T, fL, straight, fown, W, kf, frow, u, tvf, ob);
      const real* ja = W.ktab[frow][fL];
      real sq[3], cq[3];
#pragma unroll
      for (int kk = 0; kk < 3; kk++) sincos_k_small(ja[kk], &sq[kk], &cq[kk]);
      A34 Jv = J, H;
#pragma unroll
      for (int kk = 0; kk < 3; kk++)
        fk_link<true>(T, links[fL][kk], kk, Jv, H, sq[kk], cq[kk], P[kk], U[kk], kd.Jp[kk], kd.Jz[kk], kd.fp, kd.contact);
      if (dm >= 0) outer_put(outer, 0, col(dm), P, U);
      if (dp >= 0) outer_put(outer, 18, col(dp), P, U);
    }
    if (!limb) kd.contact = false;
    oc = ob;
    if (!straight) {
#pragma unroll
      for (int j = 0; j < 6; j++) {
        const real val = j < 3 ? ob.P[j] : ob.U[j - 3];
        const real vm = lane_push(val, dm >= 0 ? dm : LG - 1), vp = lane_push(val, dp >= 0 ? dp : LG - 1);
        if (pm == 0) (j < 3 ? om.P[j] : om.U[j - 3]) = vm;
        if (pp == 0) (j < 3 ? op.P[j] : op.U[j - 3]) = vp;
      }
    }
  }
  STAMP(1);
  for (int base = E0, pass = 1; base < nreq; base += LGR, pass++) {
    const bool act = limb && base + grp < nreq;
    const int bit = nth_req(act ? base + grp : 0), gr = bit >> 1, side = bit & 1;
    const int frow = __shfl(row0, gr * LG) + 4 * side;
    const int dst = act ? gr * LG + L : -1;
    BodyS ob;
#pragma unroll
    for (int j = 0; j < 3; j++) ob.P[j] = ob.U[j] = real(0);
    __builtin_amdgcn_sched_barrier(0);
    if (act) {
      real P2[3][3], U2[3][3];
      bool nb = false;
      const hs_topo* T = opaque_s(T_);
      limb_outer(T, links[L], limb_frame(T, L, straight, kd.own, W, kf, frow, u, ttab[frow] * v, ob), W.ktab[frow][L], P2,
                 U2, nb);
      outer_put(outer, side ? 18 : 0, col(dst), P2, U2);
    }
    if (!straight) {
#pragma unroll
      for (int j = 0; j < 6; j++) {
        const real val = j < 3 ? ob.P[j] : ob.U[j - 3];
        const real vm = lane_push(val, act && side == 0 ? dst : LG - 1), vp = lane_push(val, act && side == 1 ? dst : LG - 1);
        if (pm == pass) (j < 3 ? om.P[j] : om.U[j - 3]) = vm;
        if (pp == pass) (j < 3 ? op.P[j] : op.U[j - 3]) = vp;
      }
    }
  }
  __builtin_amdgcn_sched_barrier(0);
  STAMP(2);
  if constexpr (LOOP)
    if (limb) tr.issue(W, row0, L);
  wave_sync();
  if (limb) {
    if (kd.own) {
      if (straight) {
        om = body_straight(kf.own[L][0], u, tv[0]);
        op = body_straight(kf.own[L][0], u, tv[4]);
      }
      part_dyn(mk.mass_own(L), inv, om.P, oc.P, op.P, om.U, oc.U, op.U, kd.gown);
      part_g(oc.P, o, kd.gown);
      if constexpr (FORCES)
        for (int j = 0; j < 3; j++) kd.Pown[j] = oc.P[j];
    }
    const int ol = grp * HS_LMAX + l;
#pragma unroll
    for (int kk = 0; kk < 3; kk++)
      limb_centre_link<FORCES, false>(mk, outer, ol, l, L, kk, P[kk], U[kk], kd.Jp[kk], kd.Jz[kk], kd.fp, kd.Pc[kk], o, inv, kd.g3[kk], dbg_r);
    if constexpr (LOOP) {
      tr.finish(kd);
      return;
    }
    kd.bad = W.kbad[row0 + 2][L] != 0;
    kd.big |= limb_rows_big(W.ktab[row0][L], W.ktab[row0 + 2][L], W.ktab[row0 + 4][L]);
#pragma unroll
    for (int kk = 0; kk < 3; kk++) {
      if constexpr (FORCES) break;
      kd.jvel[kk] = wrap_rate(W.ktab[row0 + 3][L][kk], W.ktab[row0 + 1][L][kk], dt);
    }
  }
}

template <bool FORCES>
__device__ __attribute__((always_inline)) inline void limb_packed_kd(
    const hs_topo* T_, real (&outer)[36][LGR * HS_LMAX], hs_link (&links)[HS_LMAX][3], const RolloutWS& W, bool straight,
    const real* u, int l, int L, int ol, int row, const real* tv, const real* o, real inv, real dt, LimbKD& kd, int dbg_r,
    bool stamp_on) {
  (void)stamp_on;
  kd.own = T_->limb_own_n[L] > 0;
  BodyS om, op, oc;
  {
    real P[3][3], U[3][3];
    const hs_topo* Ts = opaque_s(T_);
    limb_outer(Ts, links[L], limb_frame(Ts, L, straight, kd.own, W, W.kf, row, u, tv[0], om), W.ktab[row][L], P, U, kd.big);
    outer_put(outer, 0, ol, P, U);
  }
  STAMP(1);
  __builtin_amdgcn_sched_barrier(0);
  {
    real P[3][3], U[3][3];
    const hs_topo* Ts = opaque_s(T_);
    limb_outer(Ts, links[L], limb_frame(Ts, L, straight, kd.own, W, W.kf, row + 4, u, tv[4], op), W.ktab[row + 4][L], P, U,
               kd.big);
    outer_put(outer, 18, ol, P, U);
  }
  __builtin_amdgcn_sched_barrier(0);
  STAMP(2);
  {
    const hs_topo* T = opaque_s(T_);
    const A34 J = limb_frame(T, L, straight, kd.own, W, W.kf, row + 2, u, tv[2], oc);
    if (kd.own) {
      part_dyn((real)T->mass[T->limb_own[L][0]], inv, om.P, oc.P, op.P, om.U, oc.U, op.U, kd.gown);
      part_g(oc.P, o, kd.gown);
      if constexpr (FORCES)
        for (int j = 0; j < 3; j++) kd.Pown[j] = oc.P[j];
    }
    const real* ja = W.ktab[row + 2][L];
    real sq[3], cq[3];
#pragma unroll
    for (int kk = 0; kk < 3; kk++) {
      kd.big |= sincos_big(ja[kk]);
      sincos_k_small(ja[kk], &sq[kk], &cq[kk]);
    }
    A34 Jv = J, H;
#pragma unroll
    for (int kk = 0; kk < 3; kk++) {
      real P0[3], U0[3];
      fk_link<true>(T, links[L][kk], kk, Jv, H, sq[kk], cq[kk], P0, U0, kd.Jp[kk], kd.Jz[kk], kd.fp, kd.contact);
      limb_centre_link<FORCES, true>(LimbModelK<false>{T, nullptr}, outer, ol, l, L, kk, P0, U0, kd.Jp[kk], kd.Jz[kk], kd.fp, kd.Pc[kk], o,
                                     inv, kd.g3[kk], dbg_r);
    }
  }
  kd.bad = W.kbad[row + 2][L] != 0;
#pragma unroll
  for (int kk = 0; kk < 3; kk++) {
    if constexpr (FORCES) break;
    kd.jvel[kk] = wrap_rate(W.ktab[row + 3][L][kk], W.ktab[row + 1][L][kk], dt);
  }
}


template <int NM, bool FORCES, bool LOOP>
struct LimbShared {
  union {
    struct {
      real outer[36][LGR * HS_LMAX];
      hs_link links[HS_LMAX][3];
    } k;
    LimbLds<NM, FORCES> g[LGR];
  };
  __device__ hs_link (&links())[HS_LMAX][3] { return k.links; }
};
template <int NM, bool FORCES>
struct LimbShared<NM, FORCES, true> {
  union {
    struct {
      real outer[36][LGR * HS_LMAX];
    } k;
    LimbLds<NM, FORCES> g[LGR];
  };
  hs_link tl[HS_LMAX][3];
  LimbRolloutK rk;
  LimbLaneK lk[LG];
  __device__ hs_link (&links())[HS_LMAX][3] { return tl; }
};
static_assert(sizeof(LimbShared<HS_NMAX, false, true>) <= 20480, "a looping wavefront's LDS: 8 per CU's 160 KB");

struct LimbHead {
  int lane;
  int rslot, b;
  bool live;
  bool straight;
  const RolloutWS* W;
  real u[3];
};

template <class P>
__device__ inline const P* opaque_u(const P* p) {
  using cptr = const __attribute__((address_space(4))) P*;
  cptr q = (cptr)p;
  asm volatile("" : "+s"(q));
  return (const P*)q;
}

template <class P>
__device__ inline const P& opaque_k(const P& r) {
  using kptr = const __attribute__((address_space(4))) P*;
  kptr q = (kptr)&r;
  asm volatile("" : "+s"(q));
  return *(const P*)q;
}

template <int NM, bool FORCES, bool TILE, bool LOOP, class... PLAN>
__device__ __attribute__((always_inline)) inline void limb_step(LimbShared<NM, FORCES, LOOP>& sh, const hs_topo* __restrict__ T,
                                                                const hs_run_args& a0, const hs::launch_map& mp0,
                                                                const LimbHead& h, int fstep, bool stamp_on,
                                                                const PLAN&... plan) {
  (void)stamp_on;
  STAMP(23);
  int lane = h.lane;
  if constexpr (LOOP) {
    asm volatile("" : "+v"(lane));
    T = opaque_u(T);
  }
  const int grp = lane >> 3, l = lane & 7, gbase = lane & ~7, rslot = h.rslot, b = h.b;
  const int nl = T->n_limbs, nmj = T->nmj;
  const bool limb = l < nl, tlane = l == LG - 1, straight = h.straight;
  const int L = limb ? l : 0;
  const real u[3] = {h.u[0], h.u[1], h.u[2]};
  bool live = h.live;
  int tile_row = 0;
  uint32_t tile_M = 0;
  uint64_t tile_req = 0;
  if constexpr (TILE) {
    const limb_tile_entry& te = limb_tile_entry_of(plan..., fstep);
    limb_tile_slot sl;
    int first;
    if constexpr (LOOP) {
      static_assert(sizeof(limb_tile_slot) == 4 && HS_TILE_SLOTS == 8, "a slot is one word: step low, row high");
      uint32_t w[HS_TILE_SLOTS];
      __builtin_memcpy(w, te.slot, sizeof(w));
      uint32_t ws = w[0];
#pragma unroll
      for (int g = 1; g < HS_TILE_SLOTS; g++) ws = grp == g ? w[g] : ws;
      sl.step = (int16_t)(ws & 0xFFFFu);
      sl.row = (int16_t)(ws >> 16);
      first = (int16_t)(w[0] & 0xFFFFu);
    } else {
      sl = te.slot[(unsigned)grp];
      first = te.slot[0].step;
    }
    live = sl.step >= 0;
    fstep = live ? sl.step : first;
    tile_row = sl.row;
    tile_M = te.M;
    tile_req = te.req;
  }
  const RolloutWS* Wp = h.W;
  if constexpr (LOOP) Wp = opaque_u(Wp);
  const RolloutWS& W = *Wp;
  const real dt = W.st.dt;
  const real v = W.st.v;
  const real inv = real(1) / (2 * dt);
  LimbLds<NM, FORCES>& S = sh.g[grp];
  const int ol = grp * HS_LMAX + (l < HS_LMAX ? l : 0);
  const int s_glob = mp0.fused_s0 + fstep;
  int k0;
  if constexpr (TILE) {
    k0 = tile_row;
  } else {
    const int call = s_glob / mp0.fused_h;
    k0 = (int)(((int64_t)a0.k0 + (int64_t)call * mp0.fused_h) % a0.n_t) + s_glob % mp0.fused_h;
  }
  const int row0 = k0 - mp0.ktab_lo;
  const real* ttab;
  const KinFrames* kfp;
  LimbModelK<LOOP> mk{T, nullptr};
  if constexpr (LOOP) {
    ttab = sh.rk.t_tab;
    kfp = &sh.rk.kf;
    mk.k = sh.lk;
  } else {
    ttab = W.t_tab;
    kfp = &W.kf;
  }
  real tv[5];
#pragma unroll
  for (int k = 0; k < 5; k += 2) tv[k] = ttab[row0 + k] * v;
  real o[3];
  const real com0[3] = {(real)T->node[0].com[0], (real)T->node[0].com[1], (real)T->node[0].com[2]};
  if (straight) {
    for (int i = 0; i < 3; i++) o[i] = fma(tv[2], u[i], W.kf.torso[i]);
  } else {
    mulp(load34r(W.ktor[row0 + 2] + 6), com0, o);
  }
  [[maybe_unused]] const int dbg_r = dbg_row(live, b, a0.horizon, s_glob);

  real g0[6];
  {
    BodyS tb[3];
#pragma unroll
    for (int k = 0; k < 3; k++) {
      if (straight) tb[k] = body_straight(W.kf.torso, u, tv[2 * k]);
      else tb[k] = body_frame(load34r(W.ktor[row0 + 2 * k] + 6), com0);
    }
    part_dyn((real)T->mass[0], inv, tb[0].P, tb[1].P, tb[2].P, tb[0].U, tb[1].U, tb[2].U, g0);
    part_g(tb[1].P, o, g0);
  }
  STAMP(0);
  LimbKD kd;
  if constexpr (TILE) {
    limb_tile_kd<FORCES, LOOP>(T, mk, *kfp, ttab, sh.k.outer, sh.links(), W, straight, u, v, lane, nl, limb, L, live, row0, tile_M,
                               tile_req, tv, o, inv, dt, kd, dbg_r, stamp_on);
  } else if (limb) {
    limb_packed_kd<FORCES>(T, sh.k.outer, sh.k.links, W, straight, u, l, L, ol, row0, tv, o, inv, dt, kd, dbg_r, stamp_on);
  }
  STAMP(3);
  wave_sync();
  if (limb) {
#pragma unroll
    for (int kk = 0; kk < 3; kk++)
      for (int j = 0; j < 6; j++) S.g[mk.node(L, kk)][j] = kd.g3[kk][j];
    if (kd.own)
      for (int j = 0; j < 6; j++) S.g[mk.own_node(L)][j] = kd.gown[j];
    if constexpr (FORCES) {
#pragma unroll
      for (int kk = 0; kk < 3; kk++)
        for (int j = 0; j < 3; j++) S.p[mk.node(L, kk)][j] = kd.Pc[kk][j];
      if (kd.own)
        for (int j = 0; j < 3; j++) S.p[mk.own_node(L)][j] = kd.Pown[j];
    }
  } else if (tlane) {
    for (int j = 0; j < 6; j++) S.g[0][j] = g0[j];
  }
  wave_sync();

  STAMP(4);
  real xt[3][3];
  if (limb) {
#pragma unroll
    for (int kk = 0; kk < 3; kk++) {
      real F[3] = {0, 0, 0}, V[3] = {0, 0, 0};
#pragma unroll
      for (int m = kk; m < 3; m++)
        for (int j = 0; j < 3; j++) { F[j] += kd.g3[m][j]; V[j] += kd.g3[m][3 + j]; }
      opaque_vals<3>(F);
      opaque_vals<3>(V);
      real d[3];
      for (int j = 0; j < 3; j++) d[j] = kd.Jp[kk][j] - o[j];
      V[0] -= d[1] * F[2] - d[2] * F[1];
      V[1] -= d[2] * F[0] - d[0] * F[2];
      V[2] -= d[0] * F[1] - d[1] * F[0];
      for (int j = 0; j < 3; j++) xt[kk][j] = V[j];
      opaque_vals<3>(xt[kk]);
      LDBG(dbg_r, T->limb_node[L][kk], V[0], 4);
      LDBG(dbg_r, T->limb_node[L][kk], F[0], 18);
      LDBG(dbg_r, T->limb_node[L][kk], d[0], 17);
    }
  }
  {
    const int nk = T->node[0].nkids;
    if (l < nk && l < HS_CMAX) {
      const int c = mk.kid(l), sz = mk.kid_size(l, c);
      real Fk[3] = {0, 0, 0}, Vk[3] = {0, 0, 0};
#pragma unroll
      for (int r = 0; r < 8; r++)
        if (r < sz)
          for (int j = 0; j < 3; j++) { Fk[j] += S.g[c + r][j]; Vk[j] += S.g[c + r][3 + j]; }
      for (int r = 8; r < sz; r++)
        for (int j = 0; j < 3; j++) { Fk[j] += S.g[c + r][j]; Vk[j] += S.g[c + r][3 + j]; }
      for (int j = 0; j < 3; j++) { S.g[c][j] = Fk[j]; S.g[c][3 + j] = Vk[j]; }
    }
  }
  wave_sync();
  if (tlane) {
    real F[3], V[3];
    for (int j = 0; j < 3; j++) { F[j] = S.g[0][j]; V[j] = S.g[0][3 + j]; }
    const int nk = T->node[0].nkids;
    for (int kk = 0; kk < HS_CMAX; kk++) {
      if (kk >= nk) break;
      const int c = T->node[0].kids[kk];
      for (int j = 0; j < 3; j++) { F[j] += S.g[c][j]; V[j] += S.g[c][3 + j]; }
    }
    const real d[3] = {0, 0, 0};
    V[0] -= d[1] * F[2] - d[2] * F[1];
    V[1] -= d[2] * F[0] - d[0] * F[2];
    V[2] -= d[0] * F[1] - d[1] * F[0];
    for (int j = 0; j < 3; j++) { S.a[j] = F[j]; S.a[3 + j] = V[j]; }
  }
  wave_sync();

  STAMP(5);
  const hs_run_args& a = LOOP ? opaque_k(a0) : a0;
  const hs::launch_map& mp = LOOP ? opaque_k(mp0) : mp0;
  if constexpr (FORCES) {
    limb_forces<NM>(T, a, mp, S, limb, l, L, gbase, nl, live, b, s_glob, o, kd.Jp, kd.Jz, kd.Pc, kd.fp, xt, kd.bad, kd.big);
    return;
  }
  const int fiL = mk.foot(L);
  const uint32_t cm = grp_or((limb && kd.contact) ? 1u << fiL : 0u);
  const int nc = __popc(cm);
  const bool mine = limb && kd.contact;
  if (limb) LDBG(dbg_r, 24 + fiL, kd.fp[2], 25);
  const int src = rank_limb(T, cm, nl, l) + gbase;
  const bool slot = l < nc;
  bool defer = grp_any(kd.big, gbase);
  bool nearf = false;
  real y3[3] = {0, 0, 0};
  real d0[3] = {0, 0, 0}, Dinv[9], gc[3], Dp6[6];
  if (mine)
    for (int r = 0; r < 3; r++) d0[r] = o[r] - kd.fp[r];
  if (mine && nc >= 2) contact_block(kd.Jp, kd.Jz, xt, kd.fp, Dp6, gc);
  if (nc >= 3) {
    float e0 = grp_getf(float(o[0] - kd.fp[0]), src), e1 = grp_getf(float(o[1] - kd.fp[1]), src),
          e2 = grp_getf(float(o[2] - kd.fp[2]), src);
    if (!slot) e0 = e1 = e2 = 0.f;
    {
      const float s0 = group8_sum(e0), s1 = group8_sum(e1), s2 = group8_sum(e2);
      const float q00 = group8_sum(e0 * e0), q11 = group8_sum(e1 * e1), q22 = group8_sum(e2 * e2);
      const float q01 = group8_sum(e0 * e1), q02 = group8_sum(e0 * e2), q12 = group8_sum(e1 * e2);
      const float k = float(nc);
      const float c00 = k * q00 - s0 * s0, c11 = k * q11 - s1 * s1, c22 = k * q22 - s2 * s2;
      const float c01 = k * q01 - s0 * s1, c02 = k * q02 - s0 * s2, c12 = k * q12 - s1 * s2;
      const float c2 = (c00 * c11 - c01 * c01) + (c00 * c22 - c02 * c02) + (c11 * c22 - c12 * c12);
      const float tq = q00 + q11 + q22;
      const float md = fmaxf(k, fmaxf(tq - q00, fmaxf(tq - q11, tq - q22)));
      const float t = kZerothGuard * k * (c00 + c11 + c22) * md;
      const bool well = c2 >= t;
      const bool nearz = c2 >= t / float(kNearBand) && c2 <= t * float(kNearBand);
      defer |= !well;
      nearf |= nearz;
    }
    STAMP(6);
    real sch[27];
#pragma unroll
    for (int e = 0; e < 27; e++) sch[e] = 0;
    bool lnear = false, ok = true;
    if (mine) {
      const real* Dp = Dp6;
      opaque_vals<3>(d0);
      const real D[9] = {Dp[0], Dp[1], Dp[3], Dp[1], Dp[2], Dp[4], Dp[3], Dp[4], Dp[5]};
      LDBG(dbg_r, 24 + fiL, Dp[0], 6);
      LDBG(dbg_r, 24 + fiL, gc[0], 7);
      real Lm[9];
      for (int i = 0; i < 9; i++) Lm[i] = D[i];
      real rl[3];
      ok = ldl_n<3>(Lm, kFastPivotGuard, rl, lnear);
      if (ok) {
        for (int j = 0; j < 3; j++) {
          real e[3] = {0, 0, 0};
          e[j] = 1;
          ldl_solve_n<3>(Lm, rl, e);
          for (int i = 0; i < 3; i++) Dinv[3 * i + j] = e[i];
        }
#pragma unroll
        for (int r = 0; r < 6; r++) {
          real E[3];
#pragma unroll
          for (int j = 0; j < 3; j++) {
            real acc = 0;
#pragma unroll
            for (int i = 0; i < 3; i++) acc += a_entry(d0, r, i) * Dinv[3 * i + j];
            E[j] = acc;
          }
// ... 74 lines not shown
        for (int r = 0; r < 6; r++) bv[i] -= a_entry(dd, r, i) * a[r];
      }
      real rl[3];
      if (mine) LDBG(dbg_r, 24 + fiL, M[4], 19);
      if (mine) LDBG(dbg_r, 24 + fiL, bv[1], 20);
      ok = chol_n<3>(M, kFastPivotGuard, rl, lnear);
      if (ok) chol_solve_n<3>(M, rl, bv);
      for (int i = 0; i < 3; i++) y[i] = bv[i];
      if (mine && ok) LDBG(dbg_r, 24 + fiL, bv[0], 21);
    } else {
      real f0[3], f1[3], dA[2][3], Dc[2][6], gg[2][3];
      for (int r = 0; r < 3; r++) {
        f0[r] = grp_get(kd.fp[r], s0);
        f1[r] = grp_get(kd.fp[r], s1);
        dA[0][r] = grp_get(d0[r], s0);
        dA[1][r] = grp_get(d0[r], s1);
        gg[0][r] = grp_get(gc[r], s0);
        gg[1][r] = grp_get(gc[r], s1);
      }
      for (int e = 0; e < 6; e++) {
        Dc[0][e] = grp_get(Dp6[e], s0);
        Dc[1][e] = grp_get(Dp6[e], s1);
      }
      const real Dm[2][9] = {{Dc[0][0], Dc[0][1], Dc[0][3], Dc[0][1], Dc[0][2], Dc[0][4], Dc[0][3], Dc[0][4], Dc[0][5]},
                             {Dc[1][0], Dc[1][1], Dc[1][3], Dc[1][1], Dc[1][2], Dc[1][4], Dc[1][3], Dc[1][4], Dc[1][5]}};
      real u[3], un = 0;
      for (int r = 0; r < 3; r++) { u[r] = f0[r] - f1[r]; un += u[r] * u[r]; }
      un = sqrt(un);
      ok = un > real(1e-12);
      real nv[6], M[36], bv[6], rl[6];
      if (ok) {
        for (int r = 0; r < 3; r++) { nv[r] = u[r] / un / sqrt(real(2)); nv[3 + r] = -nv[r]; }
        const bool first = mine && __popc(cm & ((1u << fiL) - 1)) == 0;
        if (first) LDBG(dbg_r, 24 + fiL, nv[2], 26);
        for (int i = 0; i < 6; i++) {
          const real* di = dA[i / 3];
          for (int j = 0; j < 6; j++) {
            const real* dj = dA[j / 3];
            real sv = 0;
            for (int r = 0; r < 6; r++) sv += a_entry(di, r, i % 3) * a_entry(dj, r, j % 3);
            M[6 * i + j] = sv + nv[i] * nv[j];
          }
          real sv = 0;
          for (int r = 0; r < 6; r++) sv += a_entry(di, r, i % 3) * a[r];
          bv[i] = -sv;
        }
        if (first) LDBG(dbg_r, 24 + fiL, M[5], 27);
        opaque_vals<36>(M);
        opaque_vals<6>(bv);
        opaque_vals<6>(nv);
        ok = chol_n<6>(M, kFastPivotGuard, rl, lnear);
      }
      if (ok) {
        chol_solve_n<6>(M, rl, bv);
        opaque_vals<6>(bv);
        real nDn = 0, nr = 0;
        for (int c = 0; c < 2; c++)
          for (int i = 0; i < 3; i++) {
            real Dw = 0, Dn = 0;
            for (int j = 0; j < 3; j++) { Dw += Dm[c][3 * i + j] * bv[3 * c + j]; Dn += Dm[c][3 * i + j] * nv[3 * c + j]; }
            nr += nv[3 * c + i] * (Dw + gg[c][i]);
            nDn += nv[3 * c + i] * Dn;
          }
        ok = nDn > 0;
        if (ok) {
          real t = -nr / nDn;
          for (int i = 0; i < 6; i++) y[i] = bv[i] + t * nv[i];
          if (mine && __popc(cm & ((1u << fiL) - 1)) == 0) {
            LDBG(dbg_r, 24 + fiL, y[0], 22);
            LDBG(dbg_r, 24 + fiL, bv[0], 23);
            LDBG(dbg_r, 24 + fiL, t, 24);
          }
        }
      }
    }
    defer |= !ok;
    nearf |= lnear;
    if (mine && ok) {
      const int rk = __popc(cm & ((1u << fiL) - 1));
      for (int i = 0; i < 3; i++) y3[i] = rk == 0 ? y[i] : y[3 + i];
      opaque_vals<3>(y3);
    }
  }
  STAMP(8);
  if (defer) {
    limb_defer(mp, live, l, s_glob, mp.limb_slots ? mp.limb_slots[rslot] : b);
    return;
  }

  const size_t orow = (size_t)b * a.horizon + s_glob;
  bool nan = false;
  if (limb) {
#pragma unroll
    for (int kk = 0; kk < 3; kk++) {
      const int hh = mk.hinge(L, kk);
      real d[3], yy[3];
#pragma unroll
      for (int rr = 0; rr < 3; rr++) {
        d[rr] = kd.Jp[kk][rr] - kd.fp[rr];
        yy[rr] = mine ? y3[rr] : real(0);
      }
      real tq = real(0);
#pragma unroll
      for (int r = 0; r < 3; r++) {
        real s = real(0);
#pragma unroll
        for (int jj = 0; jj < 3; jj++)
          if (jj != r) s = s + cross_e(d, jj, r) * yy[jj];
        real xr = xt[kk][r] + s;
        tq = tq + kd.Jz[kk][r] * xr;
      }
      real dw = tq * kd.jvel[kk];
      S.wd[hh] = (dw > 0) ? dw : 0;
      nan |= tq != tq;
      if (live && a.tau) outp(a.tau)[orow * mp.st_tau + hh] = tq;
    }
    if (mine)
      for (int j = 0; j < 3; j++) nan |= y3[j] != y3[j];
    if (live && a.cf)
      for (int j = 0; j < 3; j++) {
        real zv = -real(0);
        if (mine) zv = -(real(0) + (real(-1)) * y3[j]);
        outp(a.cf)[orow * mp.st_cf + 3 * fiL + j] = zv;
      }
  }
  if (live && mp.limb_rollouts) {
    if (a.tau)
      for (int c = nmj + l; c < mp.st_tau; c += LG) outp(a.tau)[orow * mp.st_tau + c] = real(0);
    if (a.cf)
      for (int c = 3 * T->nf + l; c < mp.st_cf; c += LG) outp(a.cf)[orow * mp.st_cf + c] = real(0);
  }
  const bool any_nan = grp_any(nan, gbase), any_bad = grp_any(limb && kd.bad, gbase);
  wave_sync();
  if (l == 0 && live) {
    uint32_t flags = 0;
    if (nc == 0) flags |= HS_FLAG_NO_CONTACT;
    if (nc == 1) flags |= HS_FLAG_FULL_RANK;
    if (nearf) flags |= HS_FLAG_NEAR_RANK;
    if (any_nan) flags |= HS_FLAG_NAN;
    if (any_bad) flags |= HS_FLAG_UNREACH;
    if (a.flags) a.flags[orow] = flags;
    real work_dt = real(0);
    for (int jj = 0; jj < nmj; jj++) work_dt += S.wd[jj];
    reinterpret_cast<real*>(mp.fused_work)[(size_t)s_glob * a.n_rollouts + b] = work_dt;
  }
  STAMP(9);
  RSTAMP(17);
}
#ifdef HS_STAMPS
#undef HS_STAMP_GATE
#define HS_STAMP_GATE true
#endif

struct LimbTileArgs {
  const hs_topo* T0;
  hs_run_args a;
  RolloutWS* rws;
  hs::launch_map mp;
  limb_tile_desc plan;
};

template <int NM, bool FORCES, bool TILE = false, class... PLAN>
__global__ __launch_bounds__(WAVE, HS_REAL_IS_FLOAT ? HS_LIMB_WAVES_F32 : HS_LIMB_WAVES) void hs_limb_kernel(const hs_topo* __restrict__ T0, hs_run_args a,
                                                                      RolloutWS* __restrict__ rws, hs::launch_map mp, PLAN... plan) {
  static_assert(sizeof...(PLAN) == (TILE ? 1 : 0), "the tile mapping takes the launch's tile descriptor, the packed mapping nothing");
  static_assert(!TILE || (std::is_same<PLAN, limb_tile_desc>::value && ...), "LimbTileArgs holds a limb_tile_desc");
  static_assert(offsetof(LimbTileArgs, a) == 8 && offsetof(LimbTileArgs, rws) == 8 + sizeof(hs_run_args) &&
                    offsetof(LimbTileArgs, mp) == 16 + sizeof(hs_run_args) &&
                    offsetof(LimbTileArgs, plan) == 16 + sizeof(hs_run_args) + sizeof(hs::launch_map) &&
                    alignof(hs_run_args) == 8 && alignof(hs::launch_map) == 8,
                "LimbTileArgs: the kernel argument segment packs the arguments in order at their alignment");
  constexpr bool LOOP = TILE && !FORCES && !HS_REAL_IS_FLOAT;
  __shared__ LimbShared<NM, FORCES, LOOP> sh;
  int fstep = 0, q = (int)blockIdx.x;
  const int nt = TILE ? limb_tile_count(mp.fused_n) : 0, tl = LOOP ? mp.limb_tile_loop : 1;
  fused_coords((int)blockIdx.x, mp.fused_w, TILE ? HS_TILE_SLOTS * limb_tile_chunks(nt, tl) : mp.fused_n, fstep, q);
  const hs_topo* __restrict__ T = mp.limb_model ? T0 + mp.limb_model[q] : T0;
  STAMP(18);
  {
    const uint64_t* src = reinterpret_cast<const uint64_t*>(&T->link[0][0]);
    uint64_t* dst = reinterpret_cast<uint64_t*>(&sh.links()[0][0]);
    constexpr int NW = sizeof(hs_link[HS_LMAX][3]) / sizeof(uint64_t);
    for (int e = (int)threadIdx.x; e < NW; e += WAVE) dst[e] = src[e];
    if constexpr (LOOP) {
      const int l = (int)threadIdx.x;
      if (l < LG) {
        LimbLaneK e;
        e.m[0] = e.m[1] = e.m[2] = e.mown = real(0);
        e.nodes = e.hf = e.kid = e.pad_ = 0;
        if (l < T->n_limbs) {
          const bool own = T->limb_own_n[l] > 0;
          const int on = own ? T->limb_own[l][0] : 0;
#pragma unroll
          for (int kk = 0; kk < 3; kk++) {
            const int v = T->limb_node[l][kk];
            e.m[kk] = (real)T->mass[v];
            e.nodes |= (uint32_t)v << (8 * kk);
            e.hf |= (uint32_t)T->link[l][kk].hinge << (8 * kk);
          }
          if (own) e.mown = (real)T->mass[on];
          e.nodes |= (uint32_t)on << 24;
          e.hf |= (uint32_t)T->link[l][2].foot << 24;
          e.kid = (uint32_t)own << 16;
        }
        if (l < T->node[0].nkids && l < HS_CMAX) {
          const int c = T->node[0].kids[l];
          e.kid |= (uint32_t)c | (uint32_t)T->node[c].size << 8;
        }
        sh.lk[l] = e;
      }
    } else {
      wave_sync();
    }
  }
  RSTAMP(16);
  STAMP(15);
  LimbHead h;
  h.lane = (int)threadIdx.x;
  h.rslot = q * LGR + (TILE ? fstep % LGR : h.lane >> 3);
  h.b = mp.limb_rollouts ? mp.limb_rollouts[h.rslot] : h.rslot;
  h.live = h.b >= 0 && h.b < a.n_rollouts;
  if (TILE && !h.live) return;
  const int bb = h.live ? h.b : (mp.limb_rollouts ? mp.limb_rollouts[q * LGR] : a.n_rollouts - 1);
  h.W = &rws[bb];
  const hs_gait_params& gp = a.params[bb];
  h.straight = (real)gp.curvature == 0 && !gp.rec_transform_flag;
  {
    const NodeK n0 = load_nodek(T, 0);
    for (int i = 0; i < 3; i++) h.u[i] = n0.Jp(i, 0);
  }
  if constexpr (LOOP) {
    {
      const real* src = h.W->t_tab;
      real* dst = sh.rk.t_tab;
      constexpr int NR = sizeof(LimbRolloutK) / sizeof(real);
      for (int e = (int)threadIdx.x; e < NR; e += WAVE) dst[e] = src[e];
      wave_sync();
    }
    const int c = fstep / LGR;
    for (int t0 = limb_tile_chunk_first(c, tl), t = t0, te = limb_tile_chunk_end(c, tl, nt); t < te; t++) {
      using kptr = const __attribute__((address_space(4))) LimbTileArgs*;
      kptr ka = (kptr)__builtin_amdgcn_kernarg_segment_ptr();
      asm volatile("" : "+s"(ka));
      const LimbTileArgs& k = *(const LimbTileArgs*)ka;
#ifdef HS_STAMPS
      const bool stamp_on = t - t0 == g_stamp_iter;
#else
      const bool stamp_on = true;
#endif
      limb_step<NM, FORCES, true, true>(sh, T, k.a, k.mp, h, t, stamp_on, k.plan);
      wave_sync();
    }
  } else {
    limb_step<NM, FORCES, TILE, false>(sh, T, a, mp, h, TILE ? fstep / LGR : fstep, true, plan...);
  }
}

}

namespace hs {

static int limb_deferred(unsigned long long* out) {
  return (int)hipMemcpyFromSymbol(out, HIP_SYMBOL(g_limb_deferred), sizeof(unsigned long long), 0,
                                  hipMemcpyDeviceToHost);
}

static int launch_limb(const hs_topo* d_topo, const hs_run_args& a, void* workspace, const launch_map& mp,
                       int32_t tile_plan, int32_t* tile_planned) {
  if (tile_planned) *tile_planned = 0;
  if (a.n_rollouts <= 0 || mp.fused_n <= 0) return 0;
  hipStream_t st = (hipStream_t)a.stream;
  RolloutWS* ws = (RolloutWS*)workspace;
  launch_map m = mp;
  m.fused_w = mp.limb_rollouts ? mp.limb_waves : (a.n_rollouts + LGR - 1) / LGR;
  m.limb_tile_loop = mp.limb_tile_loop < 1 || mp.tau_in || HS_REAL_IS_FLOAT ? 1 : mp.limb_tile_loop;
  const int wsteps = mp.limb_tile ? HS_TILE_SLOTS * limb_tile_chunks(limb_tile_count(mp.fused_n), m.limb_tile_loop) : mp.fused_n;
  const dim3 grid((unsigned)((int64_t)m.fused_w * wsteps));
  limb_tile_desc plan = {};
  if (mp.limb_tile) {
    const limb_tile_launch L = {mp.fused_n, mp.fused_s0, mp.fused_h, a.k0, a.n_t, mp.ktab_nl > 0 ? mp.ktab_nl : HS_LMAX};
    bool planned = false;
    if (!limb_tile_desc_build(L, tile_plan, plan, &planned)) return (int)hipErrorInvalidValue;
    if (tile_planned) *tile_planned = planned;
  }
  with_lds_class(mp.max_parts, [&](auto nm) {
    constexpr int NM = decltype(nm)::value;
    if (mp.tau_in) {
      if (mp.limb_tile)
        hipLaunchKernelGGL((hs_limb_kernel<NM, true, true, limb_tile_desc>), grid, dim3(WAVE), 0, st, d_topo, a, ws, m, plan);
      else
        hipLaunchKernelGGL((hs_limb_kernel<NM, true, false>), grid, dim3(WAVE), 0, st, d_topo, a, ws, m);
    } else {
      if (mp.limb_tile)
        hipLaunchKernelGGL((hs_limb_kernel<NM, false, true, limb_tile_desc>), grid, dim3(WAVE), 0, st, d_topo, a, ws, m, plan);
      else
        hipLaunchKernelGGL((hs_limb_kernel<NM, false, false>), grid, dim3(WAVE), 0, st, d_topo, a, ws, m);
    }
  });
  return (int)hipGetLastError();
}

}
```

hslabs_amd/csrc/hs_limb_tile.h:

```cpp
#pragma once

#include <stdint.h>

#if defined(__HIP__)
#define HS_TILE_FN __host__ __device__ inline
#else
#define HS_TILE_FN inline
#endif

constexpr int HS_TILE_SLOTS = 8;

HS_TILE_FN int limb_tile_count(int n) { return (n + HS_TILE_SLOTS - 1) / HS_TILE_SLOTS; }

HS_TILE_FN int limb_tile_step(int slot, int n) {
  const int n_even = (n + 1) / 2;
  if (slot < 0 || slot >= n) return -1;
  return slot < n_even ? 2 * slot : 2 * (slot - n_even) + 1;
}

HS_TILE_FN int limb_tile_chunks(int nt, int tl) {
  tl = tl < 1 ? 1 : tl;
  return (nt + tl - 1) / tl;
}
HS_TILE_FN int limb_tile_chunk_first(int c, int tl) { return c * (tl < 1 ? 1 : tl); }
HS_TILE_FN int limb_tile_chunk_end(int c, int tl, int nt) {
  const int e = limb_tile_chunk_first(c, tl) + (tl < 1 ? 1 : tl);
  return e < nt ? e : nt;
}

HS_TILE_FN int limb_tile_loop_rule(int nt, int64_t n_rollouts, int tiles, int64_t min_waves) {
  int tl = tiles < nt ? tiles : nt;
  while (tl > 1 && (int64_t)limb_tile_chunks(nt, tl) * n_rollouts < min_waves) tl--;
  if (tl < 1) return 1;
  const int nc = limb_tile_chunks(nt, tl);
  return (nt + nc - 1) / nc;
}

constexpr int HS_TILE_PLAN_STEPS = 256;

struct limb_tile_launch {
  int n, s0, h, k0, n_t, n_limbs;
};

HS_TILE_FN int limb_tile_row(const limb_tile_launch& L, int step) {
  const int s_glob = L.s0 + step, call = s_glob / L.h;
  return (int)(((int64_t)L.k0 + (int64_t)call * L.h) % L.n_t) + s_glob % L.h;
}
HS_TILE_FN void limb_tile_rows(const limb_tile_launch& L, int* row) {
  for (int i = 0; i < L.n; i++) row[i] = limb_tile_row(L, i);
}

HS_TILE_FN int limb_tile_e0(int n_limbs) {
  return n_limbs > 0 && n_limbs < HS_TILE_SLOTS ? HS_TILE_SLOTS * (HS_TILE_SLOTS - n_limbs) / n_limbs : 0;
}

HS_TILE_FN uint32_t limb_tile_request_mask(const int* row, const int16_t* slots) {
  uint32_t M = 0;
  for (int g = 0; g < HS_TILE_SLOTS; g++) {
    if (slots[g] < 0) continue;
    const int r = row[slots[g]];
    const bool shm = g > 0 && slots[g - 1] >= 0 && row[slots[g - 1]] + 2 == r;
    const bool shp = g < HS_TILE_SLOTS - 1 && slots[g + 1] >= 0 && row[slots[g + 1]] == r + 2;
    M |= (uint32_t)!shm << (2 * g) | (uint32_t)!shp << (2 * g + 1);
  }
  return M;
}
HS_TILE_FN int limb_tile_requests(const int* row, const int16_t* slots) { return __builtin_popcount(limb_tile_request_mask(row, slots)); }

HS_TILE_FN int limb_tile_req_passes(int req, int n_limbs) {
  const int over = req - limb_tile_e0(n_limbs);
  return over > 0 ? (over + HS_TILE_SLOTS - 1) / HS_TILE_SLOTS : 0;
}
HS_TILE_FN int limb_tile_passes(const int* row, int n, int n_limbs, const int16_t* step) {
  int passes = 0;
  for (int t = 0; t < limb_tile_count(n); t++)
    passes += limb_tile_req_passes(limb_tile_requests(row, step + HS_TILE_SLOTS * t), n_limbs);
  return passes;
}
HS_TILE_FN int limb_tile_passes(const limb_tile_launch& L, const int16_t* step) {
  int row[HS_TILE_PLAN_STEPS];
  limb_tile_rows(L, row);
  return limb_tile_passes(row, L.n, L.n_limbs, step);
}

HS_TILE_FN void limb_tile_parity_fill(int n, int16_t* step) {
  for (int s = 0; s < HS_TILE_SLOTS * limb_tile_count(n); s++) step[s] = (int16_t)limb_tile_step(s, n);
}

HS_TILE_FN void limb_tile_chain_fill(const int* row, int n, int16_t* step) {
  const int n_slots = HS_TILE_SLOTS * limb_tile_count(n);
  constexpr int NREC = HS_TILE_PLAN_STEPS + HS_TILE_PLAN_STEPS / HS_TILE_SLOTS;
  int16_t rem0[NREC], nxt[NREC];
  int head[HS_TILE_SLOTS], tail[HS_TILE_SLOTS], n_rem = 0, out = 0;
  for (int k = 0; k < HS_TILE_SLOTS; k++) head[k] = tail[k] = -1;
  auto push = [&](int first, int len) {
    rem0[n_rem] = (int16_t)first;
    nxt[n_rem] = -1;
    if (tail[len] < 0) head[len] = n_rem;
    else nxt[tail[len]] = (int16_t)n_rem;
    tail[len] = n_rem++;
  };
  for (int i = 0; i < n; i++) {
    if (i >= 2 && row[i - 2] + 2 == row[i]) continue;
    int len = 1;
    while (i + 2 * len < n && row[i + 2 * len - 2] + 2 == row[i + 2 * len]) len++;
    const int full = len / HS_TILE_SLOTS * HS_TILE_SLOTS;
    for (int j = 0; j < full; j++) step[out++] = (int16_t)(i + 2 * j);
    if (len > full) push(i + 2 * full, len - full);
  }
  while (out < n) {
    int cap = n - out < HS_TILE_SLOTS ? n - out : HS_TILE_SLOTS;
    while (cap > 0) {
      int len = cap < HS_TILE_SLOTS - 1 ? cap : HS_TILE_SLOTS - 1;
      while (len > 0 && head[len] < 0) len--;
      int take = len;
      if (len == 0) {
        for (len = cap + 1; head[len] < 0; len++) {}
        take = cap;
      }
      const int r = head[len], first = rem0[r];
      head[len] = nxt[r];
      if (head[len] < 0) tail[len] = -1;
      for (int j = 0; j < take; j++) step[out++] = (int16_t)(first + 2 * j);
      if (len > take) push(first + 2 * take, len - take);
      cap -= take;
    }
  }
  for (; out < n_slots; out++) step[out] = -1;
}

HS_TILE_FN bool limb_tile_plan_rows(const int* row, int n, int n_limbs, int16_t* step, int* passes = nullptr,
                                    int* parity_passes = nullptr) {
  int16_t par[HS_TILE_PLAN_STEPS];
  limb_tile_parity_fill(n, par);
  const int pp = limb_tile_passes(row, n, n_limbs, par);
  int pc = pp;
  if (pp > 0) {
    limb_tile_chain_fill(row, n, step);
    pc = limb_tile_passes(row, n, n_limbs, step);
  }
  if (parity_passes) *parity_passes = pp;
  if (passes) *passes = pc < pp ? pc : pp;
  if (pc < pp) return true;
  for (int s = 0; s < HS_TILE_SLOTS * limb_tile_count(n); s++) step[s] = par[s];
  return false;
}
HS_TILE_FN bool limb_tile_plan(const limb_tile_launch& L, int16_t* step, int* passes = nullptr,
                               int* parity_passes = nullptr) {
  if (L.n < 1 || L.n > HS_TILE_PLAN_STEPS || L.h < 1 || L.n_t < 1 || L.k0 < 0 || L.s0 < 0) return false;
  int row[HS_TILE_PLAN_STEPS];
  limb_tile_rows(L, row);
  return limb_tile_plan_rows(row, L.n, L.n_limbs, step, passes, parity_passes);
}

constexpr int HS_TILE_DESC_TILES = HS_TILE_PLAN_STEPS / HS_TILE_SLOTS;

struct alignas(4) limb_tile_slot {
  int16_t step;
  int16_t row;
};
struct limb_tile_entry {
  limb_tile_slot slot[HS_TILE_SLOTS];
  uint32_t M;
  uint32_t nreq;
  uint64_t req;
};
struct limb_tile_desc {
  int32_t n_tiles;
  int32_t pad_;
  limb_tile_entry tile[HS_TILE_DESC_TILES];
};
static_assert(sizeof(limb_tile_entry) == 48, "a tile's descriptor: 8 slots of 4 bytes, M, nreq and the request list");
static_assert(sizeof(limb_tile_desc) == 8 + 48 * HS_TILE_DESC_TILES && sizeof(limb_tile_desc) <= 1600,
              "the descriptor travels by value: with the kernel's other arguments well under 4 KB");

HS_TILE_FN bool limb_tile_desc_ok(int n, int h, int k0, int n_t) {
  return n >= 1 && n <= HS_TILE_PLAN_STEPS && h >= 1 && n_t >= 1 && k0 >= 0 && (int64_t)n_t + h <= 32767;
}

HS_TILE_FN void limb_tile_entry_fill(const int* row, const int16_t* slots, limb_tile_entry& e) {
  const int first = slots[0] >= 0 ? row[slots[0]] : 0;
  for (int g = 0; g < HS_TILE_SLOTS; g++) {
    e.slot[g].step = (int16_t)(slots[g] >= 0 ? slots[g] : -1);
    e.slot[g].row = (int16_t)(slots[g] >= 0 ? row[slots[g]] : first);
  }
  e.M = limb_tile_request_mask(row, slots);
  e.nreq = 0;
  e.req = 0;
// ... 34 lines not shown
```

hslabs_amd/csrc/hs_step_base.h:

```cpp
#pragma once
#include <hip/hip_runtime.h>

#include <cfloat>
#include <cstdint>
#include <type_traits>

#ifndef HS_REAL_IS_FLOAT
#define HS_REAL_IS_FLOAT 0
#endif
#include "hs_internal.h"
#include "hs_math.h"

namespace {

using namespace hsd;

#ifndef HS_CURVED_LDS
#define HS_CURVED_LDS HS_REAL_IS_FLOAT
#endif
#ifndef HS_PRELOAD
#define HS_PRELOAD (!HS_REAL_IS_FLOAT)
#endif
#ifndef HS_KTE_PRELOAD
#define HS_KTE_PRELOAD (!HS_REAL_IS_FLOAT)
// ... 96 lines not shown
  FastL fl;
  real y[HS_KMAX];
};

template <int NM, bool FORCES>
struct OneStore {
  union {
    StencilL<NM> sten;
    typename std::conditional<FORCES, ForceL, PostL<NM>>::type post;
  };
  CentreL<NM> c;
};

struct SetupL {
  real pos0[HS_LMAX][3];
  real ts[HS_LMAX], xs[HS_LMAX];
  real t_step, max_radius, v, dt;
  SC3 tsc;
};

constexpr int KT_W = 3;
constexpr int KR_W = 18;
constexpr int BF_W = 9;
struct KinFrames {
  real J0[HS_LMAX][12];
  real own[HS_LMAX][HS_OWN_MAX][BF_W];
  real torso[6];
};
__device__ inline void store_body(const A34& A, const real* com, real* bf, int n) {
  real p[3];
  mulp(A, com, p);
  for (int i = 0; i < 3; i++) bf[i] = p[i];
  bf[3] = (A(2, 1) - A(1, 2)) / 2;
  bf[4] = (A(0, 2) - A(2, 0)) / 2;
  bf[5] = (A(1, 0) - A(0, 1)) / 2;
  if (n > 6)
    for (int i = 0; i < 3; i++) bf[6 + i] = A(i, 3);
}

template <int NM>
struct SolveXY {
  union {
    real f[6 * NM];
    real x[6 * NM];
  };
  real y[HS_KMAX];
};
struct SolveNone {};
template <int NM, bool FORCES>
struct SolveL {
  typename std::conditional<FORCES, SolveXY<NM>, SolveNone>::type xy;
  int cfoot[HS_LMAX];
  uint32_t fch[HS_LMAX][2];
};
struct SolveRef {
  real* f;
  real* x;
  real* y;
  int* cfoot;
  uint32_t (*fch)[2];
};

template <int NM, bool FORCES>
struct Smem {
  OneStore<NM, FORCES> d;
  SolveL<NM, FORCES> sv;
#if HS_CURVED_LDS
  SetupL st;
#endif
};

__device__ inline void wave_sync() {
  __builtin_amdgcn_fence(__ATOMIC_RELEASE, "workgroup", "local");
  __builtin_amdgcn_s_barrier();
  __builtin_amdgcn_fence(__ATOMIC_ACQUIRE, "workgroup", "local");
}
constexpr real kNearBand = real(4);
template <class T>
__device__ inline bool near_thr(T v, T t, T band) { return v >= t / band && v <= t * band; }

__device__ inline real* outp(double* p) { return reinterpret_cast<real*>(p); }
__device__ inline const real* inp(const double* p) { return reinterpret_cast<const real*>(p); }

template <class G>
__device__ inline void gsync() {
  if constexpr (G::SHARED) wave_sync();
  else __syncthreads();
}

#ifdef HS_STAMPS
__device__ unsigned long long g_stamps[4096][32];
__device__ unsigned int g_stamp_base;
__device__ int g_stamp_iter;
#define HS_STAMP_GATE true
#define STAMP(slot)                                                                                    \
  do {                                                                                                 \
    const unsigned r_ = blockIdx.x - g_stamp_base;                                                     \
    if (threadIdx.x == 0 && r_ < 4096u && (HS_STAMP_GATE)) g_stamps[r_][slot] = __builtin_amdgcn_s_memtime(); \
  } while (0)
#define RSTAMP(slot)                                                                                   \
  do {                                                                                                 \
    const unsigned r_ = blockIdx.x - g_stamp_base;                                                     \
    if (threadIdx.x == 0 && r_ < 4096u) g_stamps[r_][slot] = __builtin_amdgcn_s_memrealtime();         \
  } while (0)
#else
#define STAMP(slot) do {} while (0)
#define RSTAMP(slot) do {} while (0)
#endif

#ifdef HS_DBG
__device__ double g_dbg[1 << 22];
__device__ inline int* dbg_rows() {
  __shared__ int r[8];
  return r;
}
#define DBG(slot, val, n)                                                        \
  do {                                                                           \
    if (HS_DBG == (n)) {                                                         \
      const int r_ = dbg_rows()[threadIdx.x / HALF];                             \
      if (r_ >= 0 && (size_t)r_ * 32 + (slot) < (1u << 22)) g_dbg[(size_t)r_ * 32 + (slot)] = (double)(val); \
    }                                                                            \
  } while (0)
#else
#define DBG(slot, val, n) do {} while (0)
#endif

__device__ inline uint32_t half_ballot(bool pred) {
  return (uint32_t)(__ballot(pred) >> (threadIdx.x & HALF));
}

__device__ inline A34 node_joint_parent(const hs_topo* T, int v) { return load34(T->node[v].J_A_parent); }
__device__ inline A34 node_pj(const hs_topo* T, int v) { return load34(T->node[v].A_pj_body); }

template <int NM, bool FORCES>
struct OneWin {
  OneStore<NM, FORCES>* d;
  __device__ bool want_pos(int k) const { return (k & 1) == 0; }
  __device__ bool want_ust(int k) const { return (k & 1) == 0; }
  __device__ bool want_q(int k) const { return k >= -1 && k <= 1; }
  __device__ bool want_centre(int k) const { return k == 0; }
  __device__ real* pos(int k, int v) const { return k == 0 ? d->c.pos[v] : d->sten.pos[k > 0][v]; }
  __device__ real* ust(int k, int v) const { return d->sten.ust[(k + 2) >> 1][v]; }
  __device__ real* q(int k) const { return d->c.q[k + 1]; }
  __device__ real* jpos(int, int v) const { return d->c.jpos[v]; }
  __device__ real* jz(int, int v) const { return d->c.jz[v]; }
  __device__ real* fpos(int, int f) const { return d->c.fpos[f]; }
  __device__ int& contact(int, int f) const { return d->c.contact[f]; }
  __device__ int& unreach(int, int L) const { return d->c.unreach[L]; }
};

#ifndef HS_KTAB
#define HS_KTAB 64
#endif
struct RolloutWS {
  SolveWS sol;
  SetupL st;
  real t_tab[HS_KTAB];
  KinFrames kf;
  real ktab[HS_KTAB][HS_LMAX][KT_W];
  real ktor[HS_KTAB][KR_W];
  uint8_t kbad[HS_KTAB][HS_LMAX];
  real kvel[HS_KTAB][HS_LMAX][KT_W];
  uint8_t kbig[HS_KTAB][HS_LMAX];
};
static_assert(sizeof(SetupL) % sizeof(real) == 0, "SetupL is copied as reals");

constexpr int kFusedGroup = 256;
__device__ inline void fused_coords(int blk, int W, int n, int& fstep, int& wid) {
  const int q = blk / (kFusedGroup * n), g0 = q * kFusedGroup;
  const int gw = W - g0 < kFusedGroup ? W - g0 : kFusedGroup;
  const int r = blk - g0 * n;
  fstep = r / gw;
  wid = g0 + r % gw;
}

}

namespace hs {

template <class F>
inline void with_lds_class(int max_parts, F&& f) {
  if (max_parts <= 18) f(std::integral_constant<int, 18>{});
  else if (max_parts <= 22) f(std::integral_constant<int, 22>{});
  else f(std::integral_constant<int, HS_NMAX>{});
}

}
```

include/hslabs.h:

```cpp
#ifndef HSLABS_H
#define HSLABS_H
#include <stddef.h>
#include <stdint.h>
#ifdef __cplusplus
extern "C" {
#endif

#define HSLABS_ABI_VERSION 16

enum {
  HS_OK = 0,
  HS_E_ARG = -1,
  HS_E_IO = -2,
  HS_E_PARSE = -3,
  HS_E_TOPOLOGY = -4,
  HS_E_NOLIK = -5,
  HS_E_DEVICE = -6,
  HS_E_NOTFOUND = -7
};

#define HS_FLAG_RANK_RETRY   1u
#define HS_FLAG_FULL_RANK    2u
#define HS_FLAG_LOOP_EXHAUST 4u
#define HS_FLAG_NAN          8u
// ... 233 lines not shown
  int32_t check_from;
  int32_t check_until;
  int32_t reserved;
  double torque_limit;
  double hc;
  const double* kick_dv;
  int32_t* state;
  double* fall_z;
} hs_sim_trial_args;

int hs_sim_trial(hs_model_t model, const hs_sim_trial_args* args);

typedef struct {
  int32_t running, survived, fallen;
  int32_t min_fall_tsi;
  int64_t sum_fall_tsi;
} hs_trial_summary;

int hs_sim_trial_summary(const int32_t* state, int32_t n, hs_trial_summary* out_host, void* stream);


int hs_sim_config(hs_model_t model, int32_t n, const double* body, double* config, int32_t config_stride,
                  int32_t precision, void* stream);

int hs_sim_track_push(hs_model_t model, int32_t n, const double* config, int32_t config_stride, double dt,
                      double* ders, int32_t precision, void* stream);

typedef struct {
  int32_t n_rollouts;
  int32_t m;
  int32_t precision;
  int32_t reserved;
  hs_sim_params params;
  const double* body;
  uint32_t* seed;
  const double* tau0;
  const double* dtau;
  double* config_out;
  double* tau_out;
  double* body_out;
  int32_t* n_contacts;
  void* stream;
} hs_sim_probe_args;

int hs_sim_probe(hs_model_t model, const hs_sim_probe_args* args);

int hs_sim_regress_B(hs_model_t model, int32_t n, int32_t m, const double* T, const double* U, double* Bt,
                     int32_t* rank, int32_t precision, void* stream);

typedef struct {
  hs_sim_probe_args probe;
  double* ders;
  double* U;
  double* Bt;
  int32_t* rank;
  void* workspace;
  size_t workspace_bytes;
} hs_sim_estimate_args;

size_t hs_sim_estimate_workspace(hs_model_t model, int32_t n_rollouts, int32_t m);

int hs_sim_estimate_B(hs_model_t model, const hs_sim_estimate_args* args);

#define HS_CPC_FLAG_NONFINITE 1u
#define HS_CPC_FLAG_NOSCORE 2u
#define HS_CPC_FLAG_RANK 4u

typedef struct {
  double w;
  double sg;
  double k0;
  double kc;
  double tauc;
  double loss_cc;
  double tp_dist;
  int32_t n_cand;
  int32_t goal_t0s;
  int32_t tpdist_switch;
  uint32_t mask;
} hs_cpc_params;

void hs_cpc_default_params(hs_cpc_params* p);

typedef struct {
  int32_t n_rollouts;
  int32_t n_tp;
  int32_t precision;
  int32_t reserved;
  hs_cpc_params params;
  const double* Bt;
  const double* state;
  int64_t state_stride;
  const double* tp;
  int64_t tp_stride;
  int32_t* low_tpdist;
  double* tau;
  int32_t* last_tpi;
  uint32_t* flags;
  double* loss;
  int32_t* cand_tpi;
  double* cand_t0s;
  int32_t* passes;
  int32_t* i_best;
  void* stream;
} hs_cpc_args;

int hs_cpc_torques(hs_model_t model, const hs_cpc_args* args);

int hs_cpc_target_points(hs_model_t model, int32_t n_rollouts, int32_t n_t, const double* q_tab, const double* dq_tab,
                         const double* tau_tab, uint32_t mask, double* tp, void* stream);

typedef struct {
  hs_sim_trial_args trial;
  hs_cpc_params cpc;
  int32_t m;
  int32_t n_tp;
  const double* dtau;
  int64_t dtau_step_stride;
  const double* tp;
  int64_t tp_stride;
  double* ders;
  double* tau0;
  int32_t* low_tpdist;
  int32_t* last_tpi;
  uint32_t* flags;
  int32_t* rank;
  void* workspace;
  size_t workspace_bytes;
} hs_sim_cpc_args;

size_t hs_sim_cpc_workspace(hs_model_t model, int32_t n_rollouts, int32_t m);

int hs_sim_cpc_step(hs_model_t model, const hs_sim_cpc_args* args);

typedef struct hs_sim_s* hs_sim_t;
int hs_sim_create(hs_model_t model, const hs_gait_params* params, int32_t n_rollouts, const hs_sim_params* sim_params,
                  double t0, hs_sim_t* out);
int hs_sim_advance(hs_sim_t sim, int32_t n_steps, double* tau_cmd, double* q_meas, double* torso, int32_t* n_contacts,
                   double* normal_force);
int hs_sim_get_state(hs_sim_t sim, double* body, int32_t* tsi);
int hs_sim_set_trial(hs_sim_t sim, int32_t open_loop, double torque_limit, int32_t kick_every, int32_t kick_phase,
                     const double* kick_dv_host, double hc, int32_t check_from, int32_t check_until);
int hs_sim_get_trial_state(hs_sim_t sim, int32_t* state_host);
void hs_sim_free(hs_sim_t sim);

int hs_model_limb_lane(hs_model_t model, int32_t* ok);
int64_t hs_limb_launches(void);
int64_t hs_limb_tile_launches(void);
int64_t hs_limb_tile_plan_launches(void);
int64_t hs_limb_tile_loop_launches(void);
int hs_limb_stats(int64_t* launches, int64_t* deferred);
int hs_debug_limb_tables(hs_model_t model, void* stream, int32_t rollout, int32_t n_rows, double* ktab, double* kvel,
                         uint8_t* kbig, uint8_t* kbad, double* dt);

const char* hs_last_error(void);
int hs_abi_version(void);

#ifdef __cplusplus
}
#endif
#endif
```

Before: 1.103 billion.

## Precompute per-limb forward kinematics rows into a table read by the tile loop

Adds a separate kernel that evaluates limb forward kinematics (positions, axes, Jacobian columns, foot point) once per keyframe row, rollout and limb, and stores them as 64-byte-aligned records in a pooled device buffer. The f64 tile-loop limb kernel gets a variant that loads these records instead of recomputing the sincos and link chain at each step, used only when the step count is large enough to reuse each row many times. This is meant to remove redundant FK arithmetic from the hot per-step kernel. In exchange it adds an extra launch, global memory traffic and buffer allocation, plus debug counters and a readback API.

After: 953.7 million. -13.5%, worse.

```diff
diff --git a/hslabs_amd/api.py b/hslabs_amd/api.py
--- a/hslabs_amd/api.py
+++ b/hslabs_amd/api.py
@@ -227,6 +227,23 @@
                                                 *(out[k].ctypes.data for k in ("ktab", "kvel", "kbig", "kbad")),
                                                 ctypes.addressof(dt)), "hs_debug_limb_tables")
     out["dt"] = float(dt.value)
+    return out
+
+
+def limb_fk_table_launches() -> int:
+    return int(capi.load().hs_limb_fk_table_launches())
+
+
+def limb_fk_table_writes() -> int:
+    return int(capi.load().hs_limb_fk_table_writes())
+
+
+def limb_fk_table(model, rollout: int, n_rows: int, device=None, stream=None) -> dict:
+    raw = np.zeros((n_rows, 6, 40))
+    capi.check(capi.load().hs_debug_limb_fk_table(model.handle, _cuda_stream(device, stream), rollout, n_rows,
+                                                  raw.ctypes.data), "hs_debug_limb_fk_table")
+    out = {k: raw[:, :, 9 * i:9 * i + 9].reshape(n_rows, 6, 3, 3).copy() for i, k in enumerate(("P", "U", "Jp", "Jz"))}
+    out["fp"] = raw[:, :, 36:39].copy()
     return out
 
 
diff --git a/hslabs_amd/capi.py b/hslabs_amd/capi.py
--- a/hslabs_amd/capi.py
+++ b/hslabs_amd/capi.py
@@ -41,6 +41,7 @@
     "hs_model_lik_host", "hs_model_fk", "hs_model_fk_host", "hs_model_get_node", "hs_model_set_torso_penalty",
     "hs_model_get_torso_penalty", "hs_model_limb_lane", "hs_limb_launches", "hs_limb_tile_launches", "hs_limb_stats",
     "hs_limb_tile_plan_launches", "hs_limb_tile_loop_launches", "hs_debug_limb_tables",
+    "hs_limb_fk_table_launches", "hs_limb_fk_table_writes", "hs_debug_limb_fk_table",
 ]
 EXPORTS_B = ["hs_sim_regress_B", "hs_sim_estimate_B"]
 HS_FLAG_LIK_FAILED = 128
@@ -325,6 +326,12 @@
     L.hs_limb_tile_loop_launches.restype = ctypes.c_int64
     L.hs_debug_limb_tables.argtypes = [vp, vp, ctypes.c_int32, ctypes.c_int32, vp, vp, vp, vp, vp]
     L.hs_debug_limb_tables.restype = ctypes.c_int
+    L.hs_limb_fk_table_launches.argtypes = []
+    L.hs_limb_fk_table_launches.restype = ctypes.c_int64
+    L.hs_limb_fk_table_writes.argtypes = []
+    L.hs_limb_fk_table_writes.restype = ctypes.c_int64
+    L.hs_debug_limb_fk_table.argtypes = [vp, vp, ctypes.c_int32, ctypes.c_int32, vp]
+    L.hs_debug_limb_fk_table.restype = ctypes.c_int
     L.hs_limb_stats.argtypes = [ctypes.POINTER(ctypes.c_int64), ctypes.POINTER(ctypes.c_int64)]
     L.hs_abi_version.argtypes = []
     L.hs_abi_version.restype = ctypes.c_int
diff --git a/hslabs_amd/csrc/hs_capi.cpp b/hslabs_amd/csrc/hs_capi.cpp
--- a/hslabs_amd/csrc/hs_capi.cpp
+++ b/hslabs_amd/csrc/hs_capi.cpp
@@ -290,6 +290,8 @@
 }
 
 std::atomic<int64_t> g_limb_launches{0};
+std::atomic<int64_t> g_limb_fk_table_launches{0};
+std::atomic<int64_t> g_limb_fk_table_writes{0};
 std::atomic<int64_t> g_limb_tile_launches{0};
 std::atomic<int64_t> g_limb_tile_plan_launches{0};
 std::atomic<int64_t> g_limb_tile_loop_launches{0};
@@ -360,6 +362,23 @@
     if (end != e && *end == '\0' && tl >= 1) return (int32_t)std::min<long>(tl, HS_TILE_PLAN_STEPS);
   }
   return limb_tile_loop_rule(nt, a.n_rollouts, HS_LIMB_TILE_LOOP_TILES, HS_LIMB_TILE_LOOP_ROUNDS * HS_RESIDENT_LIMB_WAVES);
+}
+
+#ifndef HS_LIMB_FK_TABLE_MIN_STEPS
+#define HS_LIMB_FK_TABLE_MIN_STEPS 200
+#endif
+#ifndef HS_LIMB_FK_TABLE_MIN_REUSE
+#define HS_LIMB_FK_TABLE_MIN_REUSE 8
+#endif
+bool limb_fk_table(const hs::launch_map& mp, const hs_run_args& a, bool tile, int32_t n) {
+  if (!env_switch("HS_LIMB_FK_TABLE", true)) return false;
+  int32_t min_steps = HS_LIMB_FK_TABLE_MIN_STEPS, min_reuse = HS_LIMB_FK_TABLE_MIN_REUSE;
+  if (const char* e = getenv("HS_LIMB_FK_TABLE_MIN")) {
+    char* end = nullptr;
+    const long v = strtol(e, &end, 10);
+    if (end != e && *end == '\0' && v >= 1) min_steps = (int32_t)std::min<long>(v, INT32_MAX), min_reuse = 0;
+  }
+  return limb_fk_table_rule(tile, a.precision == HS_PREC_F32, mp.tau_in != nullptr, n, mp.ktab_n, min_steps, min_reuse);
 }
 
 #ifndef HS_FUSED_WAVES
@@ -424,9 +443,31 @@
   const bool barrier_ok = (B + 63) / 64 <= 1024 && env_switch("HS_FIX_BARRIER", true);
   mp.prep_unit = limb ? 8 : 2;
   mp.ktab_rates = 0;
-  for (int32_t i = 0; !online && i < n_chunks; i++)
-    mp.ktab_rates |= limb_tile(rt, a, (int32_t)std::min<int64_t>(CHUNK, S - (int64_t)i * CHUNK)) ? 1 : 0;
+  mp.ktab_fk = 0;
+  for (int32_t i = 0; !online && i < n_chunks; i++) {
+    const int32_t n = (int32_t)std::min<int64_t>(CHUNK, S - (int64_t)i * CHUNK);
+    const bool tile = limb_tile(rt, a, n);
+    mp.ktab_rates |= tile ? 1 : 0;
+    mp.ktab_fk |= limb_fk_table(mp, a, tile, n) ? 1 : 0;
+  }
+  mp.kfk = nullptr;
+  const bool fk_reserve = rt == step_route::LIMB_FUSED && a.precision != HS_PREC_F32 && !mp.tau_in && mp.ktab_n > 0 &&
+                          (int64_t)mp.ktab_n * HS_LIMB_FK_TABLE_MIN_REUSE <= HS_FUSED_MAX_STEPS &&
+                          env_switch("HS_LIMB_FK_TABLE", true);
+  if (mp.ktab_fk || fk_reserve) {
+    const int32_t nl = mp.ktab_nl > 0 ? mp.ktab_nl : HS_LMAX;
+    std::lock_guard<std::mutex> lk(cx.pools->mu);
+    const int32_t rows = std::max<int32_t>(mp.ktab_fk ? mp.ktab_n : 0, fk_reserve ? HS_FUSED_MAX_STEPS / HS_LIMB_FK_TABLE_MIN_REUSE : 0);
+    const hipError_t e = (hipError_t)cx.pools->fused_fk.get(
+        a.stream, ((size_t)B * rows * nl * hs::HS_FK_ROW_BYTES + gwb - 1) / gwb, &mp.kfk);
+    if (e != hipSuccess) return hip_fail(e, "hipMalloc(row table)");
+    if (mp.ktab_fk) cx.pools->fk_rows = mp.ktab_n, cx.pools->fk_nl = nl;
+  }
   int le = launch_setup(cx, c, mp);
+  if (le == 0 && mp.ktab_fk) {
+    le = k.launch_limb_fk(cx.d_topo, c, cx.ws, mp);
+    g_limb_fk_table_writes++;
+  }
   mp.red_total_mass = cx.total_mass;
   mp.red_rollout_mass = cx.rollout_mass;
   mp.red_key_steps = r.key_steps;
@@ -442,6 +483,7 @@
     mp.fix_reduce = 0;
     mp.limb_tile = limb_tile(rt, a, mp.fused_n);
     mp.limb_tile_loop = mp.limb_tile ? limb_tile_loop(a, mp.fused_n) : 1;
+    mp.limb_fk = mp.ktab_fk && limb_fk_table(mp, a, mp.limb_tile != 0, mp.fused_n);
     hipError_t e = kernel_events ? hipEventRecord((hipEvent_t)kernel_events[2 * i], st) : hipSuccess;
     if (e != hipSuccess) return hip_fail(e, "hipEventRecord");
     int32_t planned = 0;
@@ -450,6 +492,7 @@
     g_limb_launches += limb;
     g_limb_tile_launches += mp.limb_tile;
     g_limb_tile_plan_launches += planned;
+    g_limb_fk_table_launches += limb && mp.limb_fk;
     g_limb_tile_loop_launches += mp.limb_tile && std::min(mp.limb_tile_loop, limb_tile_count(mp.fused_n)) > 1;
     if (le != 0) break;
     mp.fix_mode = hs::FIX_SOLVE;
@@ -498,6 +541,8 @@
 int64_t hs_limb_tile_launches(void) { return g_limb_tile_launches.load(); }
 int64_t hs_limb_tile_plan_launches(void) { return g_limb_tile_plan_launches.load(); }
 int64_t hs_limb_tile_loop_launches(void) { return g_limb_tile_loop_launches.load(); }
+int64_t hs_limb_fk_table_launches(void) { return g_limb_fk_table_launches.load(); }
+int64_t hs_limb_fk_table_writes(void) { return g_limb_fk_table_writes.load(); }
 
 int hs_limb_stats(int64_t* launches, int64_t* deferred) {
   if (launches) *launches = g_limb_launches.load();
@@ -526,6 +571,29 @@
   if (!ws) return fail(HS_E_ARG, "no workspace of this model, device and stream holds that rollout");
   e = (hipError_t)hs::limb_tables_read(ws, rollout, n_rows, ktab, kvel, kbig, kbad, dt, stream);
   if (e != hipSuccess) return hip_fail(e, "hs_debug_limb_tables");
+  return HS_OK;
+}
+
+int hs_debug_limb_fk_table(hs_model_t m, void* stream, int32_t rollout, int32_t n_rows, double* kfk) {
+  if (!m) return fail(HS_E_ARG, "null argument");
+  int dev = 0;
+  hipError_t e = hipGetDevice(&dev);
+  if (e != hipSuccess) return hip_fail(e, "hipGetDevice");
+  const char* tab = nullptr;
+  int32_t rows = 0, nl = 0;
+  {
+    std::lock_guard<std::mutex> lk(m->mu);
+    rows = m->fk_rows, nl = m->fk_nl;
+    const size_t end = ((size_t)rollout + 1) * rows * nl * hs::HS_FK_ROW_BYTES;
+    for (const auto& s : m->fused_fk.live)
+      if (s.dev == dev && s.stream == stream && rollout >= 0 && rows > 0 && end <= s.n * ws_slot_bytes()) tab = (const char*)s.ptr;
+  }
+  if (!tab || n_rows < 0 || n_rows > rows) return fail(HS_E_ARG, "no row table of this model, device and stream holds those rows");
+  e = hipStreamSynchronize((hipStream_t)stream);
+  for (int32_t r = 0; e == hipSuccess && kfk && r < n_rows; r++)
+    e = hipMemcpy(kfk + (size_t)r * HS_LMAX * (hs::HS_FK_ROW_BYTES / sizeof(double)),
+                  tab + (((size_t)rollout * rows + r) * nl) * hs::HS_FK_ROW_BYTES, (size_t)nl * hs::HS_FK_ROW_BYTES, hipMemcpyDeviceToHost);
+  if (e != hipSuccess) return hip_fail(e, "hs_debug_limb_fk_table");
   return HS_OK;
 }
 
diff --git a/hslabs_amd/csrc/hs_internal.h b/hslabs_amd/csrc/hs_internal.h
--- a/hslabs_amd/csrc/hs_internal.h
+++ b/hslabs_amd/csrc/hs_internal.h
@@ -60,16 +60,20 @@
   uint64_t* red_best_key;
   int32_t ktab_n, ktab_lo, ktab_nl, ttab_n;
   int32_t ktab_rates = 0;
+  int32_t ktab_fk = 0;
+  void* kfk = nullptr;
   int32_t prep_unit;
   const int32_t *limb_model, *limb_rollouts, *limb_slots;
   int32_t limb_waves;
   int32_t limb_tile;
   int32_t limb_tile_loop;
+  int32_t limb_fk = 0;
 };
 
 size_t solve_workspace_bytes();
 int limb_tables_read(const void* workspace, int32_t rollout, int32_t n_rows, double* ktab, double* kvel, uint8_t* kbig,
                      uint8_t* kbad, double* dt, void* stream);
+constexpr size_t HS_FK_ROW_BYTES = 320;
 void ktab_range(int32_t k0, int32_t n_t, int32_t horizon, int64_t n_calls, int32_t* lo, int32_t* n_table,
                 int32_t* n_ttab);
 launch_map single_model_map(const hs_topo& t, int32_t n_rollouts);
@@ -80,6 +84,7 @@
   int (*launch_fused)(const hs_topo* d_topo, const hs_run_args& a, void* workspace, const launch_map& mp);
   int (*launch_limb)(const hs_topo* d_topo, const hs_run_args& a, void* workspace, const launch_map& mp,
                      int32_t tile_plan, int32_t* tile_planned);
+  int (*launch_limb_fk)(const hs_topo* d_topo, const hs_run_args& a, void* workspace, const launch_map& mp);
   int (*launch_fused_reduce)(const hs_run_args& a, double total_mass, const double* rollout_mass,
                              const void* work_steps, int32_t n_steps);
   int (*limb_deferred)(unsigned long long* out);
@@ -144,9 +149,11 @@
   ws_pool ws;
   ws_pool fused_gen, fused_work;
   ws_pool fused_fix;
+  ws_pool fused_fk;
+  int32_t fk_rows = 0, fk_nl = 0;
   std::mutex mu;
   void release() {
-    for (ws_pool* p : {&ws, &fused_gen, &fused_work, &fused_fix}) p->release();
+    for (ws_pool* p : {&ws, &fused_gen, &fused_work, &fused_fix, &fused_fk}) p->release();
   }
 };
 
diff --git a/hslabs_amd/csrc/hs_kernels.hip b/hslabs_amd/csrc/hs_kernels.hip
--- a/hslabs_amd/csrc/hs_kernels.hip
+++ b/hslabs_amd/csrc/hs_kernels.hip
@@ -102,7 +102,8 @@
 
 #ifndef __HIP_DEVICE_COMPILE__
 extern const kernels kernels_f64 = {general_workspace_bytes, launch_rollouts,     launch_fused,
-                                    launch_limb,             launch_fused_reduce, limb_deferred};
+                                    launch_limb,             launch_limb_fk,
+                                    launch_fused_reduce,     limb_deferred};
 #endif
 
 }
diff --git a/hslabs_amd/csrc/hs_kernels_f32.hip b/hslabs_amd/csrc/hs_kernels_f32.hip
--- a/hslabs_amd/csrc/hs_kernels_f32.hip
+++ b/hslabs_amd/csrc/hs_kernels_f32.hip
@@ -7,7 +7,8 @@
 
 #ifndef __HIP_DEVICE_COMPILE__
 extern const kernels kernels_f32 = {general_workspace_bytes, launch_rollouts,     launch_fused,
-                                    launch_limb,             launch_fused_reduce, limb_deferred};
+                                    launch_limb,             nullptr,
+                                    launch_fused_reduce,     limb_deferred};
 #endif
 
 }
diff --git a/hslabs_amd/csrc/hs_limb.h b/hslabs_amd/csrc/hs_limb.h
--- a/hslabs_amd/csrc/hs_limb.h
+++ b/hslabs_amd/csrc/hs_limb.h
@@ -60,6 +60,8 @@
   return (const hs_topo*)q;
 }
 
+__device__ inline bool foot_contact(const hs_topo* T, const real* fp) { return fp[2] < (real)(T->rcap + 1e-4); }
+
 template <bool CENTRE>
 __device__ __attribute__((always_inline)) inline void fk_link(const hs_topo* T, const hs_link& lk, int kk, A34& Jv,
                                                               A34& H, real s, real c, real* P, real* U, real* Jp,
@@ -87,7 +89,7 @@
     if (kk == 2) {
       const real cp[3] = {(real)lk.cap[0], (real)lk.cap[1], (real)lk.cap[2]};
       mulp(H, cp, fp);
-      contact = fp[2] < (real)(T->rcap + 1e-4);
+      contact = foot_contact(T, fp);
     }
   }
 }
@@ -182,6 +184,21 @@
   bool nc = false;
 #pragma unroll
   for (int kk = 0; kk < 3; kk++) fk_link<false>(T, LK[kk], kk, Jv, H, sq[kk], cq[kk], P[kk], U[kk], nul, nul, nul, nc);
+}
+
+__device__ __attribute__((always_inline)) inline void limb_fk_row(const hs_topo* T, const hs_link (&LK)[3], int fL,
+                                                                  bool straight, bool fown, const RolloutWS& W,
+                                                                  const KinFrames& kf, int frow, const real* u, real tvf,
+                                                                  real (&P)[3][3], real (&U)[3][3], real (&Jp)[3][3],
+                                                                  real (&Jz)[3][3], real* fp, bool& contact, BodyS& ob) {
+  const A34 J = limb_frame(T, fL, straight, fown, W, kf, frow, u, tvf, ob);
+  const real* ja = W.ktab[frow][fL];
+  real sq[3], cq[3];
+#pragma unroll
+  for (int kk = 0; kk < 3; kk++) sincos_k_small(ja[kk], &sq[kk], &cq[kk]);
+  A34 Jv = J, H;
+#pragma unroll
+  for (int kk = 0; kk < 3; kk++) fk_link<true>(T, LK[kk], kk, Jv, H, sq[kk], cq[kk], P[kk], U[kk], Jp[kk], Jz[kk], fp, contact);
 }
 
 __device__ __attribute__((always_inline)) inline void outer_put(real (&outer)[36][LGR * HS_LMAX], int o0, int col,
@@ -554,15 +571,7 @@
       const hs_topo* T = opaque_s(T_);
       const bool fown = LimbModelK<LOOP>{T, mk.k}.own(fL);
       const real tvf = LOOP && limb ? tv[2] : ttab[frow] * v;
-      const A34 J = limb_frame(T, fL, straight, fown, W, kf, frow, u, tvf, ob);
-      const real* ja = W.ktab[frow][fL];
-      real sq[3], cq[3];
-#pragma unroll
-      for (int kk = 0; kk < 3; kk++) sincos_k_small(ja[kk], &sq[kk], &cq[kk]);
-      A34 Jv = J, H;
-#pragma unroll
-      for (int kk = 0; kk < 3; kk++)
-        fk_link<true>(T, links[fL][kk], kk, Jv, H, sq[kk], cq[kk], P[kk], U[kk], kd.Jp[kk], kd.Jz[kk], kd.fp, kd.contact);
+      limb_fk_row(T, links[fL], fL, straight, fown, W, kf, frow, u, tvf, P, U, kd.Jp, kd.Jz, kd.fp, kd.contact, ob);
       if (dm >= 0) outer_put(outer, 0, col(dm), P, U);
       if (dp >= 0) outer_put(outer, 18, col(dp), P, U);
     }
@@ -637,6 +646,73 @@
       if constexpr (FORCES) break;
       kd.jvel[kk] = wrap_rate(W.ktab[row0 + 3][L][kk], W.ktab[row0 + 1][L][kk], dt);
     }
+  }
+}
+
+__device__ __attribute__((always_inline)) inline void limb_tile_kd_tab(
+    const hs_topo* T_, const LimbModelK<true>& mk, const KinFrames& kf, real (&outer)[36][LGR * HS_LMAX],
+    const RolloutWS& W, const LimbFkRow* tab, int nli, bool straight, const real* u, int lane, bool limb, int L, bool live, int row0, uint32_t M,
+    const real* tv, const real* o, real inv, LimbKD& kd, int dbg_r, bool stamp_on) {
+  (void)dbg_r;
+  (void)stamp_on;
+  const int grp = lane >> 3, l = lane & 7;
+  const bool shm = live && !((M >> (2 * grp)) & 1);
+  const bool shp = live && !((M >> (2 * grp + 1)) & 1);
+  auto col = [](int ln) { return (ln >> 3) * HS_LMAX + (ln & 7); };
+  real P[3][3], U[3][3];
+  kd.own = limb && mk.own(L);
+  LimbTileRates tr;
+  if (limb) {
+    tr.issue(W, row0, L);
+    const LimbFkRow& c = tab[(row0 + 2) * nli + L];
+#pragma unroll
+    for (int kk = 0; kk < 3; kk++)
+#pragma unroll
+      for (int j = 0; j < 3; j++) {
+        P[kk][j] = c.P[kk][j];
+        U[kk][j] = c.U[kk][j];
+        kd.Jp[kk][j] = c.Jp[kk][j];
+        kd.Jz[kk][j] = c.Jz[kk][j];
+      }
+#pragma unroll
+    for (int j = 0; j < 3; j++) kd.fp[j] = c.fp[j];
+    const bool em = live && !shm, ep = live && !shp;
+    if (em || ep) {
+      const LimbFkRow& e = tab[(em ? row0 : row0 + 4) * nli + L];
+      outer_put(outer, em ? 0 : 18, col(lane), e.P, e.U);
+    }
+    if (em && ep) {
+      const LimbFkRow& e = tab[(row0 + 4) * nli + L];
+      outer_put(outer, 18, col(lane), e.P, e.U);
+    }
+    if (shp) outer_put(outer, 0, col(lane + LG), P, U);
+    if (shm) outer_put(outer, 18, col(lane - LG), P, U);
+    kd.contact = foot_contact(T_, kd.fp);
+  }
+  STAMP(1);
+  STAMP(2);
+  wave_sync();
+  if (limb) {
+    if (kd.own) {
+      BodyS om, op, oc;
+      if (straight) {
+        om = body_straight(kf.own[L][0], u, tv[0]);
+        oc = body_straight(kf.own[L][0], u, tv[2]);
+        op = body_straight(kf.own[L][0], u, tv[4]);
+      } else {
+        const hs_topo* T = opaque_s(T_);
+        limb_frame(T, L, false, true, W, kf, row0, u, tv[0], om);
+        limb_frame(T, L, false, true, W, kf, row0 + 2, u, tv[2], oc);
+        limb_frame(T, L, false, true, W, kf, row0 + 4, u, tv[4], op);
+      }
+      part_dyn(mk.mass_own(L), inv, om.P, oc.P, op.P, om.U, oc.U, op.U, kd.gown);
+      part_g(oc.P, o, kd.gown);
+    }
+    const int ol = grp * HS_LMAX + l;
+#pragma unroll
+    for (int kk = 0; kk < 3; kk++)
+      limb_centre_link<false, false>(mk, outer, ol, l, L, kk, P[kk], U[kk], kd.Jp[kk], kd.Jz[kk], kd.fp, kd.Pc[kk], o, inv, kd.g3[kk], dbg_r);
+    tr.finish(kd);
   }
 }
 
@@ -750,7 +826,7 @@
   return *(const P*)q;
 }
 
-template <int NM, bool FORCES, bool TILE, bool LOOP, class... PLAN>
+template <int NM, bool FORCES, bool TILE, bool LOOP, bool FKT, class... PLAN>
 __device__ __attribute__((always_inline)) inline void limb_step(LimbShared<NM, FORCES, LOOP>& sh, const hs_topo* __restrict__ T,
                                                                 const hs_run_args& a0, const hs::launch_map& mp0,
                                                                 const LimbHead& h, int fstep, bool stamp_on,
@@ -848,7 +924,12 @@
   }
   STAMP(0);
   LimbKD kd;
-  if constexpr (TILE) {
+  if constexpr (FKT) {
+    static_assert(!FKT || (LOOP && !FORCES), "the row table is the step mode's tile loop's");
+    const int nli = mp0.ktab_nl > 0 ? mp0.ktab_nl : HS_LMAX;
+    const LimbFkRow* tab = reinterpret_cast<const LimbFkRow*>(mp0.kfk) + (int64_t)b * mp0.ktab_n * nli;
+    limb_tile_kd_tab(T, mk, *kfp, sh.k.outer, W, tab, nli, straight, u, lane, limb, L, live, row0, tile_M, tv, o, inv, kd, dbg_r, stamp_on);
+  } else if constexpr (TILE) {
     limb_tile_kd<FORCES, LOOP>(T, mk, *kfp, ttab, sh.k.outer, sh.links(), W, straight, u, v, lane, nl, limb, L, live, row0, tile_M,
                                tile_req, tv, o, inv, dt, kd, dbg_r, stamp_on);
   } else if (limb) {
@@ -1229,6 +1310,9 @@
 #define HS_STAMP_GATE true
 #endif
 
+struct limb_tile_desc_fk : limb_tile_desc {};
+static_assert(sizeof(limb_tile_desc_fk) == sizeof(limb_tile_desc), "LimbTileArgs' plan is either");
+
 struct LimbTileArgs {
   const hs_topo* T0;
   hs_run_args a;
@@ -1241,13 +1325,15 @@
 __global__ __launch_bounds__(WAVE, HS_REAL_IS_FLOAT ? HS_LIMB_WAVES_F32 : HS_LIMB_WAVES) void hs_limb_kernel(const hs_topo* __restrict__ T0, hs_run_args a,
                                                                       RolloutWS* __restrict__ rws, hs::launch_map mp, PLAN... plan) {
   static_assert(sizeof...(PLAN) == (TILE ? 1 : 0), "the tile mapping takes the launch's tile descriptor, the packed mapping nothing");
-  static_assert(!TILE || (std::is_same<PLAN, limb_tile_desc>::value && ...), "LimbTileArgs holds a limb_tile_desc");
+  static_assert(!TILE || (std::is_base_of<limb_tile_desc, PLAN>::value && ...), "LimbTileArgs holds a limb_tile_desc");
+  constexpr bool FKT = (std::is_same<PLAN, limb_tile_desc_fk>::value || ...);
   static_assert(offsetof(LimbTileArgs, a) == 8 && offsetof(LimbTileArgs, rws) == 8 + sizeof(hs_run_args) &&
                     offsetof(LimbTileArgs, mp) == 16 + sizeof(hs_run_args) &&
                     offsetof(LimbTileArgs, plan) == 16 + sizeof(hs_run_args) + sizeof(hs::launch_map) &&
                     alignof(hs_run_args) == 8 && alignof(hs::launch_map) == 8,
                 "LimbTileArgs: the kernel argument segment packs the arguments in order at their alignment");
   constexpr bool LOOP = TILE && !FORCES && !HS_REAL_IS_FLOAT;
+  static_assert(!FKT || LOOP, "the row table's reader is the tile loop");
   __shared__ LimbShared<NM, FORCES, LOOP> sh;
   int fstep = 0, q = (int)blockIdx.x;
   const int nt = TILE ? limb_tile_count(mp.fused_n) : 0, tl = LOOP ? mp.limb_tile_loop : 1;
@@ -1325,11 +1411,11 @@
 #else
       const bool stamp_on = true;
 #endif
-      limb_step<NM, FORCES, true, true>(sh, T, k.a, k.mp, h, t, stamp_on, k.plan);
+      limb_step<NM, FORCES, true, true, FKT>(sh, T, k.a, k.mp, h, t, stamp_on, k.plan);
       wave_sync();
     }
   } else {
-    limb_step<NM, FORCES, TILE, false>(sh, T, a, mp, h, TILE ? fstep / LGR : fstep, true, plan...);
+    limb_step<NM, FORCES, TILE, false, false>(sh, T, a, mp, h, TILE ? fstep / LGR : fstep, true, plan...);
   }
 }
 
@@ -1341,6 +1427,82 @@
   return (int)hipMemcpyFromSymbol(out, HIP_SYMBOL(g_limb_deferred), sizeof(unsigned long long), 0,
                                   hipMemcpyDeviceToHost);
 }
+
+#if !HS_REAL_IS_FLOAT
+}
+namespace {
+constexpr int HS_FK_TPB = WAVE;
+constexpr int HS_FK_REALS = sizeof(LimbFkRow) / sizeof(real);
+__global__ __launch_bounds__(HS_FK_TPB) void hs_limb_fk_kernel(const hs_topo* __restrict__ T0, hs_run_args a,
+                                                              RolloutWS* __restrict__ rws, hs::launch_map mp) {
+  static_assert(std::is_same<real, double>::value && HS_FK_REALS == 40 && sizeof(LimbFkRow) == hs::HS_FK_ROW_BYTES,
+                "records leave as double2 pieces");
+  __shared__ real st[HS_FK_REALS][WAVE + 1];
+  __shared__ LimbFkRow* dst[WAVE];
+  const int tl = (int)threadIdx.x;
+  const int nli = mp.ktab_nl > 0 ? mp.ktab_nl : HS_LMAX, nr = mp.ktab_n;
+  const int64_t id = (int64_t)blockIdx.x * HS_FK_TPB + tl;
+  const int L = (int)(id % nli), r = (int)((id / nli) % nr);
+  const int64_t rs = id / ((int64_t)nli * nr);
+  const int64_t n_slots = mp.limb_rollouts ? (int64_t)mp.limb_waves * LGR : a.n_rollouts;
+  int b = -1;
+  if (rs < n_slots) b = mp.limb_rollouts ? mp.limb_rollouts[rs] : (int)rs;
+  bool on = b >= 0 && b < a.n_rollouts;
+  const hs_topo* __restrict__ T = on && mp.limb_model ? T0 + mp.limb_model[rs / LGR] : T0;
+  on = on && L < T->n_limbs;
+  LimbFkRow* e = nullptr;
+  if (on) {
+    RolloutWS& W = rws[b];
+    const hs_gait_params& gp = a.params[b];
+    const bool straight = (real)gp.curvature == 0 && !gp.rec_transform_flag;
+    real u[3];
+    {
+      const NodeK n0 = load_nodek(T, 0);
+      for (int i = 0; i < 3; i++) u[i] = n0.Jp(i, 0);
+    }
+    real P[3][3], U[3][3], Jp[3][3], Jz[3][3], fp[3];
+    bool contact = false;
+    BodyS ob;
+    limb_fk_row(T, T->link[L], L, straight, T->limb_own_n[L] > 0, W, W.kf, r, u, W.t_tab[r] * W.st.v, P, U, Jp, Jz, fp,
+                contact, ob);
+    e = reinterpret_cast<LimbFkRow*>(mp.kfk) + ((int64_t)b * nr + r) * nli + L;
+#pragma unroll
+    for (int kk = 0; kk < 3; kk++)
+#pragma unroll
+      for (int j = 0; j < 3; j++) {
+        st[3 * kk + j][tl] = P[kk][j];
+        st[9 + 3 * kk + j][tl] = U[kk][j];
+        st[18 + 3 * kk + j][tl] = Jp[kk][j];
+        st[27 + 3 * kk + j][tl] = Jz[kk][j];
+      }
+#pragma unroll
+    for (int j = 0; j < 3; j++) st[36 + j][tl] = fp[j];
+    st[39][tl] = real(0);
+  }
+  dst[tl] = e;
+  __syncthreads();
+  static_assert(offsetof(LimbFkRow, U) == 9 * sizeof(real) && offsetof(LimbFkRow, Jp) == 18 * sizeof(real) &&
+                    offsetof(LimbFkRow, Jz) == 27 * sizeof(real) && offsetof(LimbFkRow, fp) == 36 * sizeof(real),
+                "st's rows are LimbFkRow's values in order");
+#pragma unroll 4
+  for (int k = 0; k < HS_FK_REALS / 2; k++) {
+    const int idx = k * WAVE + tl, rec = idx / (HS_FK_REALS / 2), c = idx % (HS_FK_REALS / 2);
+    LimbFkRow* d = dst[rec];
+    if (d) *reinterpret_cast<double2*>(reinterpret_cast<real*>(d) + 2 * c) = make_double2(st[2 * c][rec], st[2 * c + 1][rec]);
+  }
+}
+}
+namespace hs {
+
+static int launch_limb_fk(const hs_topo* d_topo, const hs_run_args& a, void* workspace, const launch_map& mp) {
+  const int64_t n_slots = mp.limb_rollouts ? (int64_t)mp.limb_waves * LGR : a.n_rollouts;
+  const int64_t lanes = n_slots * mp.ktab_n * (mp.ktab_nl > 0 ? mp.ktab_nl : HS_LMAX);
+  if (lanes <= 0) return 0;
+  hipLaunchKernelGGL(hs_limb_fk_kernel, dim3((unsigned)((lanes + HS_FK_TPB - 1) / HS_FK_TPB)), dim3(HS_FK_TPB), 0,
+                     (hipStream_t)a.stream, d_topo, a, (RolloutWS*)workspace, mp);
+  return (int)hipGetLastError();
+}
+#endif
 
 static int launch_limb(const hs_topo* d_topo, const hs_run_args& a, void* workspace, const launch_map& mp,
                        int32_t tile_plan, int32_t* tile_planned) {
@@ -1368,7 +1530,13 @@
       else
         hipLaunchKernelGGL((hs_limb_kernel<NM, true, false>), grid, dim3(WAVE), 0, st, d_topo, a, ws, m);
     } else {
-      if (mp.limb_tile)
+      if (mp.limb_tile && mp.limb_fk && !HS_REAL_IS_FLOAT) {
+        if constexpr (!HS_REAL_IS_FLOAT) {
+          limb_tile_desc_fk pf;
+          static_cast<limb_tile_desc&>(pf) = plan;
+          hipLaunchKernelGGL((hs_limb_kernel<NM, false, true, limb_tile_desc_fk>), grid, dim3(WAVE), 0, st, d_topo, a, ws, m, pf);
+        }
+      } else if (mp.limb_tile)
         hipLaunchKernelGGL((hs_limb_kernel<NM, false, true, limb_tile_desc>), grid, dim3(WAVE), 0, st, d_topo, a, ws, m, plan);
       else
         hipLaunchKernelGGL((hs_limb_kernel<NM, false, false>), grid, dim3(WAVE), 0, st, d_topo, a, ws, m);
diff --git a/hslabs_amd/csrc/hs_limb_tile.h b/hslabs_amd/csrc/hs_limb_tile.h
--- a/hslabs_amd/csrc/hs_limb_tile.h
+++ b/hslabs_amd/csrc/hs_limb_tile.h
@@ -34,6 +34,10 @@
   if (tl < 1) return 1;
   const int nc = limb_tile_chunks(nt, tl);
   return (nt + nc - 1) / nc;
+}
+
+HS_TILE_FN bool limb_fk_table_rule(bool tile, bool f32, bool forces, int n, int rows, int min_steps, int min_reuse) {
+  return tile && !f32 && !forces && rows > 0 && n >= min_steps && (int64_t)n >= (int64_t)min_reuse * rows;
 }
 
 constexpr int HS_TILE_PLAN_STEPS = 256;
diff --git a/hslabs_amd/csrc/hs_step_base.h b/hslabs_amd/csrc/hs_step_base.h
--- a/hslabs_amd/csrc/hs_step_base.h
+++ b/hslabs_amd/csrc/hs_step_base.h
@@ -272,6 +272,11 @@
 #ifndef HS_KTAB
 #define HS_KTAB 64
 #endif
+struct alignas(64) LimbFkRow {
+  real P[3][3], U[3][3], Jp[3][3], Jz[3][3], fp[3], pad_;
+};
+static_assert(sizeof(LimbFkRow) % 64 == 0 && sizeof(LimbFkRow) == (sizeof(real) == 8 ? 320 : 192), "whole lines per limb lane");
+
 struct RolloutWS {
   SolveWS sol;
   SetupL st;
diff --git a/include/hslabs.h b/include/hslabs.h
--- a/include/hslabs.h
+++ b/include/hslabs.h
@@ -409,6 +409,9 @@
 int hs_limb_stats(int64_t* launches, int64_t* deferred);
 int hs_debug_limb_tables(hs_model_t model, void* stream, int32_t rollout, int32_t n_rows, double* ktab, double* kvel,
                          uint8_t* kbig, uint8_t* kbad, double* dt);
+int64_t hs_limb_fk_table_launches(void);
+int64_t hs_limb_fk_table_writes(void);
+int hs_debug_limb_fk_table(hs_model_t model, void* stream, int32_t rollout, int32_t n_rows, double* kfk);
 
 const char* hs_last_error(void);
 int hs_abi_version(void);
```
